# PytorchConnectomics/pytorch_connectomics

Hardware: AMD Instinct MI355X
Metric: voxels/s (train + sliding-window infer), MedNeXt-S 112^3 bf16 (higher is better)
Workload: dtype bf16; 1 GPU; Lucchi++ sliding-window inference (configs[1]): MedNeXt-S k3, 165x1024x768 volume, roi 112^3, overlap 0.5, bump blending, sw_batch_size 8, random-init weights; step = one whole-volume EagerSlidingWindowEngine call (TTA off); value = window-voxels/s; sw_batch_size=8, window_pipeline_streams=3

## Files before the change

include/pytc_hip.h:

```cpp
#ifndef PYTC_HIP_H
#define PYTC_HIP_H

#include <stdint.h>

#ifdef __cplusplus
extern "C" {
#endif

#define PYTC_ABI_VERSION 15

#define PYTC_OK 0
#define PYTC_ERR_INVALID 1
#define PYTC_ERR_HIP 2
#define PYTC_ERR_UNSUPPORTED 3

#define PYTC_F32 0
#define PYTC_BF16 1
#define PYTC_F16 2

#define PYTC_VIEW_FLIP_Z 1
#define PYTC_VIEW_FLIP_Y 2
#define PYTC_VIEW_FLIP_X 4
#define PYTC_VIEW_SWAP_YX 8
#define PYTC_VIEW_SWAP_ZY 16
#define PYTC_VIEW_SWAP_ZX 32

#define PYTC_PAD_CONSTANT 0
#define PYTC_PAD_REFLECT 1
#define PYTC_PAD_REPLICATE 2
#define PYTC_PAD_CIRCULAR 3

#define PYTC_BLEND_PRODUCT 0
#define PYTC_BLEND_MIN 1

#define PYTC_ACT_NONE 0
#define PYTC_ACT_SIGMOID 1
#define PYTC_ACT_TANH 2
#define PYTC_ACT_GELU 3

#define PYTC_RES_NONE 0
#define PYTC_RES_ADD 1
#define PYTC_RES_UPSAMPLE 2
#define PYTC_RES_GELU_BWD 3
#define PYTC_RES_NORM_BWD 4

int pytc_abi_version(void);
const char* pytc_last_error(void);
int pytc_device_info(int device, int* cu_count, int* lds_bytes_per_cu, char* arch, int arch_len);
int pytc_set_tuning(const char* key, int value);


int pytc_gather_windows(const float* vol, int C, int Z, int Y, int X, const int32_t* starts, int B,
                        int rz, int ry, int rx, int view, int pad_mode, float cval, void* out,
                        int out_dtype, void* stream);

int pytc_blend_accumulate(const void* pred, int pred_dtype, int B, const int32_t* starts, int rz,
                          int ry, int rx, int C, int view, const float* wz, const float* wy,
                          const float* wx, int combine, float floor_w, const int32_t* border ,
                          float* value, float* weight, int Z, int Y, int X, void* stream);

int pytc_blend_accumulate_mapped(const void* pred, int pred_dtype, int B, const int32_t* starts, int rz, int ry,
                                 int rx, int C, int view, const float* wz, const float* wy, const float* wx,
                                 int combine, float floor_w, const int32_t* border, const int32_t* chan_src,
                                 const int32_t* chan_shift, float* value, float* weight, int Z, int Y, int X,
                                 void* stream);
int pytc_blend_weight_shifted(int B, const int32_t* starts, int rz, int ry, int rx, const float* wz, const float* wy,
                              const float* wx, int combine, float floor_w, const int32_t* border,
                              const int32_t* shift, float* weight, int Z, int Y, int X, void* stream);
int pytc_normalize_covered(float* value, const float* weight, int64_t n, void* stream);
int pytc_ensemble_update_masked(float* stat, float* count, const float* x, const float* cover, int64_t n, int mode,
                                void* stream);
int pytc_ensemble_finalize_masked(const float* stat, const float* count, float* out, int64_t n, int mode, void* stream);

int pytc_blend_finalize(float* value, const float* weight, int C, int64_t nvox, float clamp,
                        int act, void* stream);

#define PYTC_ACT_SOFTMAX 4
int pytc_channel_activation(float* value, int C, int64_t nvox, int channels_last, int c0, int c1, int act,
                            float scale, void* stream);

int pytc_ensemble_update(float* acc, const float* x, int64_t n, int mode, int count, void* stream);

#define PYTC_ST_U8 0
#define PYTC_ST_I8 1
#define PYTC_ST_U16 2
#define PYTC_ST_I16 3
#define PYTC_ST_I32 4
#define PYTC_ST_F16 5
#define PYTC_ST_F32 6
int pytc_scale_cast(const float* x, void* y, int64_t n, float scale, int target, void* stream);


#define PYTC_RAW_U8 0
#define PYTC_RAW_I8 1
#define PYTC_RAW_U16 2
#define PYTC_RAW_I16 3
#define PYTC_RAW_U32 4
#define PYTC_RAW_I32 5
#define PYTC_RAW_F32 6
#define PYTC_RAW_F64 7
int pytc_resample_region(const void* raw, int raw_dtype, const int64_t* strides_czyx, int C, const int32_t* tab_i0,
                         const int32_t* tab_i1, const float* tab_f, const int32_t* dims_zyx, float* out, void* stream);

#define PYTC_NORM_NONE 0
#define PYTC_NORM_ZSCORE 1
#define PYTC_NORM_MINMAX 2
#define PYTC_NORM_DIVIDE 3
int64_t pytc_window_normalize_ws_elems(int B, int64_t n);
int pytc_window_normalize(float* x, int B, int64_t n, int mode, int binarize, float threshold, float divide, const float* clip,
                          double* workspace, void* stream);


int pytc_dwconv3d_stat_slots(int N, int D, int H, int W, int C, int K, int stride, int dtype,
                             int transposed);

int pytc_dwconv3d_kernel_variant(int N, int D, int H, int W, int C, int K, int stride, int dtype, int transposed);

int pytc_dwconv3d_fwd(const void* x, void* y, const float* w, const float* bias, float* stats,
                      int N, int D, int H, int W, int C, int K, int stride, int dtype,
                      void* stream);

int pytc_dwconv3d_fwd_wide(const void* x, void* y, const float* w, const float* bias, float* stats, int N, int D, int H,
                           int W, int C, int K, int stride, int dtype, void* stream);

int pytc_dwconv3d_res_supported(int D, int H, int W, int C, int K, int stride, int dtype);

int pytc_dwmix_supported(int D, int H, int W, int C, int C_hid, int C_out, int dtype);
int pytc_dwmix_fwd(const void* x, const float* taps, const float* dw_bias, const void* w2n, const float* b2n, const void* w3_f16,
                   const float* b3, int residual, void* y, const void* head_w, const float* head_b, float* head_y, int n_head, int N,
                   int D, int H, int W, int C, int C_hid, int C_out, int dtype, void* stream);
int pytc_dwconv3d_fwd_res(const void* x, const void* res, void* y, const float* w, const float* bias, int N, int D, int H,
                          int W, int C, int K, int stride, int dtype, void* stream);

int pytc_dwconvT3d_fwd(const void* x, void* y, const float* w, const float* bias, float* stats,
                       int N, int D, int H, int W, int C, int K, int dtype, void* stream);

int pytc_groupnorm_finalize(const float* stats, int slots, float count, const float* gamma,
                            const float* beta, float eps, float* ab, int N, int C, void* stream);


int64_t pytc_pw_packed_elems(int C_out, int C_in, int dtype);
int pytc_pw_pack_weight(const float* w, int C_out, int C_in, int transposed, void* packed,
                        int dtype, void* stream);

typedef struct {
  const void* x;
  const void* w_packed;
  const float* bias;
  const float* ab;
  const void* res;
  void* y;
  int N;
  int64_t rows_per_sample;
  int C_in, C_out;
  int in_dtype, out_dtype, w_dtype;
  int act;
  int res_mode;
  int gather;
  int Di, Hi, Wi;
  const void* res_low;
  const float* res_bias;
  int pre_act;
  int w_paired;
} pytc_pw_args;

int pytc_pw_conv_fwd(const pytc_pw_args* a, void* stream);
int pytc_pw_conv_paired_supported(const pytc_pw_args* a);
int pytc_pw_conv_rowmajor_supported(const pytc_pw_args* a);

typedef struct {
  const void* t;
  const float* ab;
  const void* w2_packed;
  const float* b2;
  const void* w3_packed;
  const float* b3;
  const void* res;
  const void* res_low;
  const float* res_bias;
  void* y;
  int N;
  int64_t rows_per_sample;
  int C_in, C_hid, C_out;
  int res_mode;
  int Di, Hi, Wi;
  int w3_format;
  int per_sample;
} pytc_mlp_args;
#define PYTC_W3_BF16 0
#define PYTC_W3_F16 1

int pytc_pw_gemm_supported(int C_in, int C_out);
int pytc_pw_gemm_fwd(const void* x, const void* w, const float* bias, const float* ab, void* y, int N, int64_t rows_per_sample,
                     int C_in, int C_out, int in_f16, int gelu_out, const void* res, const void* res_low, const float* res_bias,
                     int res_mode, int Di, int Hi, int Wi, void* stream);
int pytc_pw_mlp_supported(int C_in, int C_hid, int C_out);
int pytc_pw_pack_weight_paired(const float* w, int C_out, int C_in, int transposed, void* packed_bf16,
                               void* stream);
int pytc_pack_multi(const int64_t* table_dev, int n_items, int64_t total_elems, void* stream);
int pytc_pw_pack_weight_paired_f16(const float* w, int C_out, int C_in, int transposed, void* packed_f16,
                                   void* stream);
int pytc_pw_mlp_fwd(const pytc_mlp_args* a, void* stream);

int pytc_pw_mlp_lds_supported(int C_in, int C_hid, int C_out);
int pytc_pw_mlp_lds_fwd(const pytc_mlp_args* a, void* stream);
int pytc_pw_mlp_dma_applies(const pytc_mlp_args* a, int ignore_res_mode);
int pytc_pw_mlp_proj_supported(int C_in, int C_hid, int C_out, int C_proj);
int pytc_pw_mlp_proj_fwd(const pytc_mlp_args* a, const void* proj_w, const float* proj_b, void* z, int store_y, void* stream);
int pytc_pw_mlp_chunk_supported(int C_in, int C_hid, int C_out);
int pytc_pw_mlp_chunk_fwd(const pytc_mlp_args* a, void* stream);
int pytc_groupnorm_fold_mlp(const float* stats, int slots, float count, const float* gamma, const float* beta, float eps,
                            const float* w2, const float* b2, void* w2n, float* b2n, float* ab_out, int N, int C, int C_hid,
                            void* stream);
int pytc_pw_mlp_train_fwd(const pytc_mlp_args* a, void* hidden_pre, void* stream);
int pytc_pw_mlp_train_fwd_nostore(const pytc_mlp_args* a, void* stream);
int pytc_pw_mlp_bwd(const pytc_mlp_args* a, const void* hidden_pre, void* d_hidden, void* stream);
int pytc_pw_mlp_up_supported(int C_in, int C_hid, int C_out);
int pytc_pw_mlp_up_fwd(const pytc_mlp_args* a, const float* taps, const float* dw_bias, void* stream);
int pytc_pw_mlp_head_supported(int C_in, int C_hid, int C_out);
int pytc_pw_mlp_stemres_fwd(const pytc_mlp_args* a, const float* stem_x, const float* stem_w, const float* stem_b,
                            void* stream);
int pytc_stem_dwconv3d_stat_slots(int D, int H, int W);
int pytc_stem_dwconv3d_supported(int C_in, int C, int K);
int pytc_stem_dwconv3d_mfma_image_bytes(void);
int pytc_stem_dwconv3d_pack_mfma(const float* wx, const float* wb, const float* cst, void* image, void* stream);
int pytc_stem_dwconv3d_fwd(const float* x, const float* wx, const float* wb, const float* cst, const void* mfma_image, void* y,
                           float* stats, int N, int D, int H, int W, int C, void* stream);
int pytc_pw_mlp_head_fwd(const pytc_mlp_args* a, const void* head_w, const float* head_b, float* head_y, int n_head,
                         int store_y, void* stream);


#define PYTC_ACT_RELU 5
#define PYTC_ACT_LEAKY 6
#define PYTC_ACT_ELU 7

typedef struct {
  const void* x;
  const void* w_packed;
  const float* bias;
  const float* ab;
  const void* res;
  void* y;
  int N, D, H, W, C_in, C_out;
  int kd, kh, kw;
  int act_in;
  float act_param;
  int res_mode;
  int dtype;
} pytc_conv3d_args;

int64_t pytc_conv3d_packed_elems(int C_out, int C_in, int kd, int kh, int kw, int dtype);
int pytc_conv3d_pack_weight(const float* w, int C_out, int C_in, int kd, int kh, int kw, void* packed, int dtype,
                            void* stream);
int pytc_conv3d_fwd(const pytc_conv3d_args* a, void* stream);

int pytc_channel_stats_slots(int64_t rows);
int pytc_channel_stats(const void* x, float* stats, int N, int64_t rows, int C, int dtype, void* stream);
int pytc_norm_finalize_groups(const float* stats, int slots, float count, const float* gamma, const float* beta,
                              float eps, int groups, float* ab, int N, int C, void* stream);
int pytc_affine_act(const void* x, void* y, const float* ab, int N, int64_t rows, int C, int act, float prm,
                    int dtype, void* stream);
int pytc_maxpool3d_fwd(const void* x, void* y, int N, int D, int H, int W, int C, int fz, int fy, int fx, int dtype,
                       void* stream);
int pytc_dwconvT3d_generic_fwd(const void* x, void* y, const float* w, int N, int D, int H, int W, int C,
                               const int32_t* kernel, const int32_t* stride, const int32_t* pad, int dtype,
                               void* stream);


int pytc_groupnorm_finalize_mr(const float* stats, int slots, float count, const float* gamma, const float* beta,
                               float eps, float* ab, float* mean_rstd, int N, int C, void* stream);
int pytc_gelu(const void* x, const void* dy, void* out, int64_t n, int dtype, void* stream);
int pytc_add_inplace(void* y, const void* x, int64_t n, int dtype, void* stream);
int pytc_pw_wgrad_slots(int64_t rows_total);
int pytc_pw_wgrad(const void* x, const float* ab, const void* dy, float* dW, float* db, float* workspace, int N,
                  int64_t rows_per_sample, int C_in, int C_out, int dtype, int x_act , void* stream);
int pytc_dw_wgrad_slots(int N, const int32_t* gdims, const int32_t* xdims, int C, int K, int stride, int dtype);
int pytc_dw_wgrad(const void* g, const void* x, float* dW, float* db, float* workspace, int N, const int32_t* gdims,
                  const int32_t* xdims, int C, int K, int stride, int dtype, void* stream);

int pytc_pw_wgrad_partial(const void* x, const float* ab, const void* dy, float* workspace, int want_db, int N,
                          int64_t rows_per_sample, int C_in, int C_out, int dtype, int x_act, int* slots_out, void* stream);
int pytc_pw_wgrad_dgrad_supported(int C_in, int C_out, int dtype);
int pytc_pw_wgrad_dgrad_partial(const void* x, const void* dy, const void* w_t_paired, void* dx, float* workspace, int want_db, int N,
                                int64_t rows_per_sample, int C_in, int C_out, int dtype, int* slots_out, void* stream);
int pytc_mixer_bwd_rc_supported(int C, int C_hid, int C_out, int dtype);
int pytc_mixer_bwd_rc_sps(int N, int64_t rows_per_sample, int C_hid);
int64_t pytc_mixer_bwd_rc_ws_elems(int N, int64_t rows_per_sample, int C_hid, int gn);
int pytc_mixer_bwd_rc(const void* t, const float* ab, const float* mean_rstd, const void* dy, const void* w2_paired, const float* b2,
                      const void* w3t_paired, const float* W2, const float* gamma, float count, void* dhp, float* workspace,
                      float* s_out, float* coef, int want_db3, int gn, int N, int64_t rows_per_sample, int C, int C_hid, int C_out,
                      int dtype, int* slots_out, void* stream);
int pytc_dw_wgrad_partial(const void* g, const void* x, float* workspace, int want_db, int N, const int32_t* gdims,
                          const int32_t* xdims, int C, int K, int stride, int dtype, int* slots_out, void* stream);
int pytc_copy_zero_front(const void* src, void* dst, int N, const int32_t* dims, int C, int dtype, void* stream);
typedef struct {
  const float* part;
  float* out;
  int64_t n;
  int32_t slots;
  int32_t out_t;
} pytc_reduce_item;
int pytc_reduce_slots_multi(const pytc_reduce_item* items, int n_items, void* stream);
int pytc_norm_bwd_ws_elems(int N, int64_t rows, int C);
int pytc_norm_bwd(const void* dtn, const void* t, const float* mean_rstd, const float* gamma, float* stats_ws,
                  float* s_out, void* dt, int N, int64_t rows, float count , int C,
                  int dtype, void* stream);
int pytc_pw_wgrad_groupnorm_supported(int C, int C_hid, int dtype);
int pytc_pw_wgrad_groupnorm_sps(int N, int64_t rows_per_sample, int C, int C_hid);
int64_t pytc_pw_wgrad_groupnorm_ws_elems(int N, int64_t rows_per_sample, int C, int C_hid);
int pytc_pw_wgrad_groupnorm(const void* t, const float* mean_rstd, const float* ab, const void* dhp, const float* W2,
                            const float* gamma, float count, float* s_out, float* coef, float* workspace, int N,
                            int64_t rows_per_sample, int C, int C_hid, int dtype, void* stream);
int pytc_norm_bwd_apply(const void* dtn, const void* t, const float* mean_rstd, const float* gamma, const float* s_in,
                        int s_parts, void* dt, int N, int64_t rows, int C, float count, int dtype, const int32_t* crop_grid,
                        void* stream);
int pytc_dwconv3d_bwd_data(const void* dy, const float* w, void* dx, int N, const int32_t* xdims,
                           const int32_t* ydims, int C, int K, int stride, int dtype, void* stream);
int pytc_dwconv3d_bwd_data_add(const void* dy, const float* w, const void* addend, void* dx, int N, const int32_t* xdims,
                               const int32_t* ydims, int C, int K, int stride, int dtype, void* stream);

int pytc_conv3d_pack_weight_dgrad(const float* w, int C_out, int C_in, int kd, int kh, int kw, void* packed, int dtype,
                                  void* stream);
int pytc_conv3d_pack_plan(int C_out, int C_in, int kd, int kh, int kw, int dtype, int direct, int64_t* out);
int pytc_conv3d_pack_multi(const int64_t* table_dev, int n_items, int64_t total_blocks, void* stream);
int pytc_conv3d_launch_plan(int N, int D, int H, int W, int C_in, int C_out, int kd, int kh, int kw, int dtype, int has_pre,
                            int has_res, int phase, int64_t* out);
int pytc_norm_bwd_means(const float* s, const float* gamma, float* M, float* dgamma, float* dbeta, int N, int C, int groups,
                        float rows, void* stream);
int pytc_bn_train_finalize_cpad(const float* stats, int slots_total, float count, const float* gamma, const float* beta, float eps,
                                float momentum, float* running_mean, float* running_var, int64_t* num_batches_tracked, float* ab,
                                float* mean_rstd, int N, int C, int C_real, void* stream);
int pytc_norm_finalize_groups_cpg(const float* stats, int slots, float count, const float* gamma, const float* beta, float eps,
                                  int groups, int cpg, float* ab, float* mr, int N, int C, void* stream);
int pytc_norm_bwd_means_cpg(const float* s, const float* gamma, float* M, float* dgamma, float* dbeta, int N, int C, int groups,
                            int cpg, float rows, void* stream);
int pytc_bn_train_finalize(const float* stats, int slots_total, float count, const float* gamma, const float* beta, float eps,
                           float momentum, float* running_mean, float* running_var, int64_t* num_batches_tracked, float* ab,
                           float* mean_rstd, int N, int C, void* stream);
int pytc_bn_update_running(const float* mean_rstd, float* running_mean, float* running_var, int C, float count, float eps,
                           float momentum, void* stream);
int64_t pytc_conv3d_wgrad_ws_elems(int N, int D, int H, int W, int C_in, int C_out, const int32_t* kernel, int dtype);
int pytc_conv3d_wgrad(const void* a, const void* dy, float* dW, float* workspace, int N, int D, int H, int W, int C_in,
                      int C_out, const int32_t* kernel, int dtype, void* stream);
int pytc_act_bwd(const void* da, const void* x, const float* ab, void* dt, void* dp, int N, int64_t rows, int C, int act,
                 float prm, int dtype, void* stream);
int pytc_norm_finalize_groups_mr(const float* stats, int slots, float count, const float* gamma, const float* beta,
                                 float eps, int groups, float* ab, float* mr, int N, int C, void* stream);
int pytc_norm_bwd_stats(const void* dtn, const void* t, const float* mean_rstd, float* stats_ws, float* s_out, int N,
                        int64_t rows, int C, int dtype, void* stream);
int pytc_norm_bwd_apply_general(const void* d, const void* x, const float* mean_rstd, const float* gamma, const float* M,
                                void* dx, int N, int64_t rows, int C, int dtype, void* stream);
int pytc_act_norm_bwd_stats(const void* da, const void* x, const float* ab, const float* mean_rstd, float* stats_ws, float* s_out,
                            float* p_ws, float* p_out, int N, int64_t rows, int C, int act, float prm, int dtype, void* stream);
int pytc_act_norm_bwd_apply(const void* da, const void* x, const float* ab, const float* mean_rstd, const float* gamma,
                            const float* M, void* dx, int N, int64_t rows, int C, int act, float prm, int dtype, void* stream);
int pytc_act_norm_bwd_apply_cg(const void* da, const void* x, const float* ab, const float* mean_rstd, const float* gamma, int C_gamma,
                               const float* M, void* dx, int N, int64_t rows, int C, int act, float prm, int dtype, void* stream);
int pytc_maxpool3d_bwd(const void* x, const void* dy, void* dx, int N, int D, int H, int W, int C, int fz, int fy, int fx,
                       int dtype, void* stream);
int pytc_dwconv3d_generic_fwd(const void* x, void* y, const float* w, int N, int D, int H, int W, int C,
                              const int32_t* kernel, const int32_t* stride, const int32_t* pad, const int32_t* out_dims,
                              int dtype, void* stream);

int64_t pytc_conv3d_direct_packed_elems(int C_out, int C_in, int kd, int kh, int kw, int dtype);
int pytc_conv3d_pack_weight_direct(const float* w, int C_out, int C_in, int kd, int kh, int kw, int64_t s_o, int64_t s_c,
                                   int flip, void* packed, int dtype, void* stream);
int pytc_convT3d_c1_fwd(const void* x, const float* w, const float* bias, void* y, float* workspace, int N, const int32_t* in_dims,
                        int C_in, int dtype, void* stream);
int pytc_convT3d_phase_plan(int C_out, int C_in, int dtype, int64_t* out);
int pytc_convT3d_phase_supported(int C_out, int C_in, int dtype);
int pytc_convT3d_phase_fwd(const pytc_conv3d_args* a, const int32_t* in_dims, void* stream);
int pytc_conv3d_strided_fwd(const pytc_conv3d_args* a, const int32_t* in_dims, const int32_t* stride, const int32_t* pad,
                            int transposed, void* stream);
int64_t pytc_conv3d_wgrad_strided_ws_elems(int N, const int32_t* small_dims, int C_k, int C_o, const int32_t* kernel);
int pytc_conv3d_wgrad_strided(const void* big, const void* small, float* dW, float* workspace, int N,
                              const int32_t* big_dims, const int32_t* small_dims, int C_k, int C_o, const int32_t* kernel,
                              const int32_t* stride, const int32_t* pad, int dtype, void* stream);
int pytc_convT3d_thin_supported(int C_in, int C_out);
int pytc_convT3d_thin_fwd(const void* x, const float* w, const float* bias, void* y, int N, const int32_t* in_dims, int C_in,
                          int C_out, int dtype, void* stream);

int pytc_layernorm_rows(const void* x, void* y, const float* gamma, const float* beta, int64_t rows, int C, float eps,
                        int dtype, void* stream);
int pytc_upcat_deconv2_fwd(const void* x_low, const float* w, const float* bias, const void* x_e, void* cat, int N, int d, int h, int wd,
                           int D, int H, int W, int C_in, int C_e, int C_u, int dtype, void* stream);
int pytc_upcat_deconv2_bwd_data(const void* dcat, const float* w, void* dx_e, void* dx_low, int N, int d, int h, int wd, int D, int H,
                                int W, int C_in, int C_e, int C_u, int dtype, void* stream);
int64_t pytc_upcat_deconv2_wgrad_ws_elems(int rows, int C_in, int C_u, int dtype);
int pytc_upcat_deconv2_wgrad(const void* x_low, const void* dcat, float* workspace, float* dw, float* db, int N, int d, int h, int wd,
                             int D, int H, int W, int C_in, int C_e, int C_u, int dtype, void* stream);
int pytc_linear_fwd(const void* x, const float* w, const float* bias, const float* pos, int pos_rows, const void* res, void* y, int M,
                    int N, int K, int x_gelu, int dtype, void* stream);
int pytc_linear_bwd_data(const void* dy, const float* w, const void* x_gelu, void* dx, int M, int N, int K, int dtype, void* stream);
int pytc_linear_wgrad(const void* dy, const void* x, float* dw, float* db, float* dpos, int pos_rows, int M, int N, int K, int x_gelu,
                      int dtype, void* stream);
int pytc_layernorm_wide(const void* x, void* y, const float* gamma, const float* beta, int64_t rows, int C, float eps, int dtype,
                        void* stream);
int pytc_layernorm_wide_bwd_slots(int64_t rows);
int pytc_layernorm_wide_bwd(const void* dy, const void* x, const float* gamma, void* dx, float* partial, float* dgamma, float* dbeta,
                            int64_t rows, int C, float eps, int dtype, void* stream);
int pytc_patch_gather16(const void* src, void* dst, int B, int D, int H, int W, int C, int scatter, int dtype, void* stream);
int pytc_attention_supported(int d_head);
int pytc_attention_fwd(const void* qkv, void* out, float* lse, int B, int N, int heads, int d_head, float scale, int dtype,
                       void* stream);
int pytc_attention_bwd(const void* qkv, const void* out, const void* dout, const float* lse, float* dvec, void* dqkv, int B, int N,
                       int heads, int d_head, float scale, int dtype, void* stream);
int pytc_window_attention_supported(int d_head);
int pytc_window_attention_bias_groups(int nwin, int N, int heads);
int pytc_window_attention_fwd(const void* qkv, const float* table, const int* geom, void* out, float* lse, int nwin, int N, int heads,
                              int d_head, float scale, int dtype, void* stream);
int pytc_window_attention_bwd(const void* qkv, const float* table, const int* geom, const void* out, const void* dout, const float* lse,
                              float* dvec, void* dqkv, float* partial, float* dtable, int nwin, int N, int heads, int d_head, float scale,
                              int dtype, void* stream);
int pytc_window_partition(const void* src, void* dst, const void* res, const int* geom, int B, int C, int reverse, int dtype,
                          void* stream);
int pytc_space_to_depth2(const void* src, void* dst, int B, int D, int H, int W, int C, int order, int scatter, int dtype, void* stream);
int pytc_layernorm_any(const void* x, void* y, const float* gamma, const float* beta, int64_t rows, int C, float eps, int dtype,
                       void* stream);
int pytc_layernorm_any_bwd_slots(int64_t rows);
int pytc_layernorm_any_bwd(const void* dy, const void* x, const float* gamma, void* dx, float* stats, float* partial, float* dgamma,
                           float* dbeta, int64_t rows, int C, float eps, int dtype, void* stream);
int pytc_deconv2_upfirst_fwd(const void* x_low, const float* w, const float* bias, const void* x_e, void* out, int N, int d, int h,
                             int wd, int C_in, int C_e, int C_u, int dtype, void* stream);
int pytc_deconv2_upfirst_bwd_data(const void* dout, const float* w, void* dx_e, void* dx_low, int N, int d, int h, int wd, int C_in,
                                  int C_e, int C_u, int dtype, void* stream);
int pytc_deconv2_upfirst_wgrad(const void* x_low, const void* dout, float* workspace, float* dw, float* db, int N, int d, int h, int wd,
                               int C_in, int C_e, int C_u, int dtype, void* stream);
int pytc_layernorm_rows_bwd_slots(int64_t rows, int C, int dtype);
int pytc_layernorm_rows_bwd(const void* dy, const void* x, const float* gamma, void* dx, float* partial, int64_t rows, int C,
                            float eps, int dtype, void* stream);
int pytc_grn_bwd_apply(const void* dh2, const void* hp, const float* A, const float* B, void* out, int N, int64_t rows, int C,
                       int dtype, void* stream);
int64_t pytc_bce_dice_ws_elems(int N, int C, int64_t R);
int pytc_bce_dice_fwd(const float* logits, const float* target, const float* weight, int N, int C, int64_t R,
                      const int64_t* x_strides, const int64_t* t_strides, const int64_t* w_strides, float pos_weight,
                      float w_bce, float w_dice, float smooth_nr, float smooth_dr, float* workspace, float* sums,
                      float* out, void* stream);
int pytc_bce_dice_bwd(const float* logits, const float* target, const float* weight, const float* sums, const float* out,
// ... 124 lines not shown
```

pytorch_connectomics_amd/csrc/dwconvT_tile_kernels.hip:

```cpp
#include <mutex>

#include "dwconv_march.h"

namespace pytc {

constexpr int TT_TZ = 2, TT_TX = 8;

template <int C, int TY, bool STORE>
__global__ void __launch_bounds__(256, 4)
dwconvT3d_k3_tile_kernel(const unsigned short* __restrict__ x, unsigned short* __restrict__ y, const float* __restrict__ w,
                         const float* __restrict__ bias, float* __restrict__ stats, DwTTile g) {
  constexpr int LPV = C / 2;
  constexpr int SLOTS = 256 / LPV;
  constexpr int CELLS = TT_TZ * TY * TT_TX;
  constexpr int EZ = TT_TZ + 1, EY = TY + 1, EX = TT_TX + 1;
  constexpr int NCH = EZ * EY * EX * (C / 8);
  typedef unsigned int u32x4_t __attribute__((ext_vector_type(4)));
  extern __shared__ __attribute__((aligned(16))) unsigned short tile[];
  unsigned short* const otile = tile + EZ * EY * EX * C + (threadIdx.x >> 6) * 1024;
  __shared__ float red[256 / 64][2][2 * 64];

  const int tid = threadIdx.x;
  int b = blockIdx.x;
  const int fx = b % g.tx; b /= g.tx;
  const int fy = b % g.ty;
  const int fz = b / g.ty;
  const int n = blockIdx.y;
  const int z0 = fz * TT_TZ, y0 = fy * TY, x0 = fx * TT_TX;
  const long vcells = (long)g.D * g.H * g.W;
  const unsigned short* xn = x + (long)n * vcells * C;
  unsigned short* yn = y + (long)n * vcells * 8 * C;
  const int Ho = 2 * g.H, Wo = 2 * g.W;

  constexpr int LPT = (NCH + 255) / 256;
  u32x4_t st[LPT];
#pragma unroll
  for (int i = 0; i < LPT; ++i) {
    const int c = tid + 256 * i;
    const int vox = c / (C / 8), part = c % (C / 8);
    const int lx = vox % EX, t = vox / EX;
    const int ly = t % EY, lz = t / EY;
    const int iz = min(max(z0 - 1 + lz, 0), g.D - 1), iy = min(max(y0 - 1 + ly, 0), g.H - 1), ix = min(max(x0 - 1 + lx, 0), g.W - 1);
    if (c < NCH) st[i] = *reinterpret_cast<const u32x4_t*>(xn + (((long)iz * g.H + iy) * g.W + ix) * C + part * 8);
  }
  const int pr = tid % LPV, slot0 = tid / LPV;
  float wt[27][2];
#pragma unroll
  for (int t = 0; t < 27; ++t) {
    const float2 v = *reinterpret_cast<const float2*>(w + (long)t * C + pr * 2);
    wt[t][0] = v.x; wt[t][1] = v.y;
  }
  float bv[2] = {0.f, 0.f};
  if (bias) { bv[0] = bias[pr * 2]; bv[1] = bias[pr * 2 + 1]; }
#pragma unroll
  for (int i = 0; i < LPT; ++i) {
    const int c = tid + 256 * i;
    if (c < NCH) *reinterpret_cast<u32x4_t*>(tile + (long)c * 8) = st[i];
  }
  __syncthreads();

  typedef __bf16 bf2_t __attribute__((ext_vector_type(2)));
  typedef float f2_t __attribute__((ext_vector_type(2)));
  const unsigned int SX = 2u * C * 2u, SY = (unsigned int)Wo * C * 2u * 2u, SZ = (unsigned int)Ho * Wo * C * 2u * 2u;
  char* const ybase = reinterpret_cast<char*>(yn) + ((((long)2 * z0 * Ho + 2 * y0) * Wo + 2 * x0) * C) * 2;
  const int lane = tid & 63;
  int pcs[2];
  unsigned int poff[2];
#pragma unroll
  for (int k = 0; k < 2; ++k) {
    const int piece = lane + 64 * k, vox = piece / (C / 8), chunk = piece % (C / 8);
    const int q = vox % 8;
    pcs[k] = vox / 8;
    poff[k] = (unsigned int)(q >> 2) * (SZ / 2) + (unsigned int)((q >> 1) & 1) * (SY / 2) + (unsigned int)(q & 1) * (SX / 2) + chunk * 16u;
  }
  const int wslot0 = (tid >> 6) * (64 / LPV);
  f2_t s1 = {0.f, 0.f}, s2 = {0.f, 0.f};
  const bool interior = z0 > 0 && y0 > 0 && x0 > 0 && z0 + TT_TZ <= g.D && y0 + TY <= g.H && x0 + TT_TX <= g.W;
  const f2_t bv2 = {bv[0], bv[1]};
  f2_t wt2[27];
#pragma unroll
  for (int t = 0; t < 27; ++t) wt2[t] = f2_t{wt[t][0], wt[t][1]};
  for (int it = 0; it < CELLS / SLOTS; ++it) {
    const int cell = slot0 + it * SLOTS;
    const int cx = cell % TT_TX, t = cell / TT_TX;
    const int cy = t % TY, cz = t / TY;
    const int mz = z0 + cz, my = y0 + cy, mx = x0 + cx;
    const bool live = interior || (mz < g.D && my < g.H && mx < g.W);
    f2_t xin[2][2][2];
#pragma unroll
    for (int a = 0; a < 2; ++a)
#pragma unroll
      for (int bb = 0; bb < 2; ++bb)
#pragma unroll
        for (int d = 0; d < 2; ++d) {
          const unsigned int v = *reinterpret_cast<const unsigned int*>(tile + ((((cz + a) * EY + cy + bb) * EX + cx + d) * C + pr * 2));
          xin[a][bb][d] = f2_t{__uint_as_float(v << 16), __uint_as_float(v & 0xffff0000u)};
        }
    const bool fz0 = !interior && mz == 0, fy0 = !interior && my == 0, fx0 = !interior && mx == 0;
    unsigned int* const orow = reinterpret_cast<unsigned int*>(otile) + ((slot0 - wslot0) * 8) * (C / 2) + pr;
#pragma unroll
    for (int pz = 0; pz < 2; ++pz)
#pragma unroll
      for (int py = 0; py < 2; ++py)
#pragma unroll
        for (int px = 0; px < 2; ++px) {
          f2_t acc = bv2;
#pragma unroll
          for (int a = pz; a < 2; ++a)
#pragma unroll
            for (int bb = py; bb < 2; ++bb)
#pragma unroll
              for (int d = px; d < 2; ++d) {
                const int kz = pz ? 1 : (a ? 0 : 2), ky = py ? 1 : (bb ? 0 : 2), kx = px ? 1 : (d ? 0 : 2);
                acc = __builtin_elementwise_fma(xin[a][bb][d], wt2[(kz * 3 + ky) * 3 + kx], acc);
              }
          const bool zero = !live || (pz == 0 && fz0) || (py == 0 && fy0) || (px == 0 && fx0);
          unsigned int bits = __builtin_bit_cast(unsigned int, __builtin_convertvector(acc, bf2_t));
          bits = zero ? 0u : bits;
          if (STORE) orow[(pz * 4 + py * 2 + px) * (C / 2)] = bits;
          const f2_t r = {__uint_as_float(bits << 16), __uint_as_float(bits & 0xffff0000u)};
          s1 += r;
          s2 = __builtin_elementwise_fma(r, r, s2);
        }
    if (STORE) {
      __builtin_amdgcn_wave_barrier();
#pragma unroll
      for (int k = 0; k < 2; ++k) {
        const u32x4_t o = *reinterpret_cast<const u32x4_t*>(otile + (lane + 64 * k) * 8);
        const int c2 = wslot0 + pcs[k] + it * SLOTS;
        const int c2x = c2 % TT_TX, t2 = c2 / TT_TX;
        const int c2y = t2 % TY, c2z = t2 / TY;
        const bool ok = interior || (z0 + c2z < g.D && y0 + c2y < g.H && x0 + c2x < g.W);
        const unsigned int off = __umul24((unsigned int)c2z, SZ) + __umul24((unsigned int)c2y, SY) + (unsigned int)c2x * SX + poff[k];
        if (ok) *reinterpret_cast<u32x4_t*>(ybase + off) = o;
      }
      __builtin_amdgcn_wave_barrier();
    }
  }
  if (stats) {
    if (LPV == 32) {
#pragma unroll
      for (int i = 0; i < 2; ++i) { s1[i] += __shfl_xor(s1[i], 32, 64); s2[i] += __shfl_xor(s2[i], 32, 64); }
    }
    const int wave = tid >> 6, lane = tid & 63;
    if (lane < LPV) {
      red[wave][0][(lane % LPV) * 2] = s1[0]; red[wave][0][(lane % LPV) * 2 + 1] = s1[1];
      red[wave][1][(lane % LPV) * 2] = s2[0]; red[wave][1][(lane % LPV) * 2 + 1] = s2[1];
    }
    __syncthreads();
    if (tid < 2 * C) {
      const int which = tid / C, ch = tid % C;
      float a = 0.f;
#pragma unroll
      for (int wv = 0; wv < 4; ++wv) a += red[wv][which][ch];
      stats[(((long)n * g.slots + blockIdx.x) * 2 + which) * C + ch] = a;
    }
  }
}

bool dwconvT_tile_plan(DwTTile& g, int N, int D, int H, int W, int C) {
  if (C != 64 && C != 128) return false;
  const int ty = C == 64 ? 8 : 4;
  g.N = N; g.D = D; g.H = H; g.W = W; g.C = C;
  g.tz = (D + TT_TZ - 1) / TT_TZ; g.ty = (H + ty - 1) / ty; g.tx = (W + TT_TX - 1) / TT_TX;
  g.slots = g.tz * g.ty * g.tx;
  return g.slots >= 1 && (long)D * H * W * 8 * C * 2 < (1L << 32) && (long)(2 * H) * (2 * W) * C * 4 < (1L << 24);
}

void dwconvT_tile_launch(const void* x, void* y, const float* w, const float* bias, float* stats, const DwTTile& g, hipStream_t s) {
  dim3 grid((unsigned)g.slots, (unsigned)g.N), block(256);
  const unsigned short* xp = (const unsigned short*)x;
  unsigned short* yp = (unsigned short*)y;
#define PYTC_TT(CC, TYY, ST)                                                                                                  \
  do {                                                                                                                        \
    if (!ensure_dynamic_lds(reinterpret_cast<const void*>(&dwconvT3d_k3_tile_kernel<CC, TYY, ST>), 64 * 1024, "dwconvT3d_k3_tile")) return; \
    hipLaunchKernelGGL((dwconvT3d_k3_tile_kernel<CC, TYY, ST>), grid, block,                                                  \
                       (size_t)(TT_TZ + 1) * (TYY + 1) * (TT_TX + 1) * CC * 2 + 4 * 2048, s, xp, yp, w, bias, stats, g);                  \
  } while (0)
  if (g.C == 64) { if (y) PYTC_TT(64, 8, true); else PYTC_TT(64, 8, false); }
  else { if (y) PYTC_TT(128, 4, true); else PYTC_TT(128, 4, false); }
#undef PYTC_TT
}

}
```

pytorch_connectomics_amd/csrc/dwconv_march.h:

```cpp
#pragma once
#include "pytc_common.h"

namespace pytc {

struct DwMarch {
  int N, D, H, W, C;
  int ty, tx, zc, nzc;
  int tilex;
  int slots;
  int swizzle;
  int cg_inner;
};

void dwconv_mfma_launch(const void* x, void* y, const float* w, const float* bias, float* stats, const DwMarch& g, int variant,
                        hipStream_t s);

struct DwMix {
  const bf16x8_t* w2n;
  const float* b2n;
  const h8_t* w3;
  const float* b3;
  long w2_stride;
  int residual;
  const bf16x8_t* head_w;
  const float* head_b;
  float* head_y;
  int n_head, store_y;
};
int dwmix_launch(const void* x, void* y, const float* w, const float* bias, const DwMarch& g, const DwMix& mx, int c_hid, int variant,
                 hipStream_t s);

struct DwTTile { int N, D, H, W, C, tz, ty, tx, slots; };
bool dwconvT_tile_plan(DwTTile& g, int N, int D, int H, int W, int C);
void dwconvT_tile_launch(const void* x, void* y, const float* w, const float* bias, float* stats, const DwTTile& g, hipStream_t s);

struct DwS2 { int N, D, H, W, C, Do, Ho, Wo, ty, tx, zc, nzc, slots; };
bool dwconv_s2_plan(DwS2& g, int N, int D, int H, int W, int C);
void dwconv_s2_launch(const void* x, void* y, const float* w, const float* bias, float* stats, const DwS2& g, hipStream_t s);

}
```

pytorch_connectomics_amd/csrc/dwconv_s2_kernels.hip:

```cpp
#include <mutex>

#include "dwconv_march.h"

namespace pytc {

constexpr int S2_TYO = 4;

template <int C>
__global__ void __launch_bounds__(256, 2)
dwconv3d_k3_s2_march_kernel(const unsigned short* __restrict__ x, unsigned short* __restrict__ y, const float* __restrict__ w,
                            const float* __restrict__ bias, float* __restrict__ stats, DwS2 g) {
  constexpr int TYO = S2_TYO, TXO = 8, IY = 2 * TYO + 1, IX = 2 * TXO + 1;
  constexpr int LPV = C / 2, VS = 256 / LPV, OUTV = TYO * TXO, ITEMS = OUTV / VS;
  constexpr int PCH = IY * IX * (C / 8);
  constexpr int LPT = (PCH + 255) / 256;
  constexpr int PLANE = IY * IX * C;
  typedef unsigned int u32x4_t __attribute__((ext_vector_type(4)));
  typedef float f2_t __attribute__((ext_vector_type(2)));
  typedef __bf16 bf2_t __attribute__((ext_vector_type(2)));
  constexpr int OPIECES = OUTV * C / 8;
  static_assert(OUTV % VS == 0 && OPIECES <= 256, "at most one 16-byte output piece per thread and plane");
  extern __shared__ __attribute__((aligned(16))) unsigned short ring[];
  unsigned short* const otile = ring + 3 * PLANE;
  __shared__ float red[4][2][2 * 64];

  const int tid = threadIdx.x;
  int b = blockIdx.x;
  const int fx = b % g.tx; b /= g.tx;
  const int fy = b % g.ty;
  const int zchunk = b / g.ty;
  const int n = blockIdx.y;
  const int yo0 = fy * TYO, xo0 = fx * TXO;
  const int zs = zchunk * g.zc, ze = min(zs + g.zc, g.Do);
  const long in_plane = (long)g.H * g.W * C;
  const unsigned short* xn = x + (long)n * g.D * in_plane;
  unsigned short* yn = y + (long)n * g.Do * g.Ho * g.Wo * C;

  int goff[LPT], loff[LPT];
  bool cok[LPT];
#pragma unroll
  for (int i = 0; i < LPT; ++i) {
    const int c = tid + 256 * i;
    const int vox = c / (C / 8), part = c % (C / 8);
    const int lx = vox % IX, ly = vox / IX;
    const int iy = 2 * yo0 - 1 + ly, ix = 2 * xo0 - 1 + lx;
    cok[i] = c < PCH && iy >= 0 && iy < g.H && ix >= 0 && ix < g.W;
    goff[i] = (min(max(iy, 0), g.H - 1) * g.W + min(max(ix, 0), g.W - 1)) * C + part * 8;
    loff[i] = c < PCH ? c * 8 : -1;
  }
  auto request = [&](int iz, u32x4_t (&st)[LPT]) {
    const unsigned short* src = xn + (long)min(max(iz, 0), g.D - 1) * in_plane;
#pragma unroll
    for (int i = 0; i < LPT; ++i) st[i] = *reinterpret_cast<const u32x4_t*>(src + goff[i]);
  };
  auto deposit = [&](int iz, const u32x4_t (&st)[LPT]) {
    const bool zok = iz >= 0 && iz < g.D;
    unsigned short* dst = ring + ((iz + 1) % 3) * PLANE;
#pragma unroll
    for (int i = 0; i < LPT; ++i)
      if (loff[i] >= 0) *reinterpret_cast<u32x4_t*>(dst + loff[i]) = (zok && cok[i]) ? st[i] : u32x4_t{0u, 0u, 0u, 0u};
  };

  const int pr = tid % LPV, vslot = tid / LPV;
  f2_t wt[27];
#pragma unroll
  for (int t = 0; t < 27; ++t) {
    const float2 v = *reinterpret_cast<const float2*>(w + (long)t * C + pr * 2);
    wt[t] = f2_t{v.x, v.y};
  }
  f2_t bv = {0.f, 0.f};
  if (bias) bv = f2_t{bias[pr * 2], bias[pr * 2 + 1]};
  const int ovx = tid / (C / 8), opart = tid % (C / 8);
  const int oyy = yo0 + ovx / TXO, oxx = xo0 + ovx % TXO;
  const bool ook = tid < OPIECES && oyy < g.Ho && oxx < g.Wo;
  const long obase = ((long)oyy * g.Wo + oxx) * C + opart * 8;

  u32x4_t sa[LPT], sb[LPT];
  request(2 * zs - 1, sa);
  request(2 * zs, sb);
  deposit(2 * zs - 1, sa);
  deposit(2 * zs, sb);
  request(2 * zs + 1, sa);
  deposit(2 * zs + 1, sa);
  __syncthreads();

  f2_t s1 = {0.f, 0.f}, s2 = {0.f, 0.f};
  for (int zo = zs; zo < ze; ++zo) {
    const bool more = zo + 1 < ze;
    if (more) { request(2 * zo + 2, sa); request(2 * zo + 3, sb); }
    const unsigned short* p0 = ring + ((2 * zo) % 3) * PLANE;
    const unsigned short* p1 = ring + ((2 * zo + 1) % 3) * PLANE;
    const unsigned short* p2 = ring + ((2 * zo + 2) % 3) * PLANE;
#pragma unroll
    for (int it = 0; it < ITEMS; ++it) {
      const int v = vslot + it * VS;
      const int vy = v / TXO, vx = v % TXO;
      const int base = ((2 * vy) * IX + 2 * vx) * C + pr * 2;
      f2_t acc = bv;
#pragma unroll
      for (int kz = 0; kz < 3; ++kz) {
        const unsigned short* pl = kz == 0 ? p0 : (kz == 1 ? p1 : p2);
#pragma unroll
        for (int ky = 0; ky < 3; ++ky)
#pragma unroll
          for (int kx = 0; kx < 3; ++kx) {
            const unsigned int u = *reinterpret_cast<const unsigned int*>(pl + base + (ky * IX + kx) * C);
            acc = __builtin_elementwise_fma(f2_t{__uint_as_float(u << 16), __uint_as_float(u & 0xffff0000u)}, wt[(kz * 3 + ky) * 3 + kx], acc);
          }
      }
      const bool live = (yo0 + vy) < g.Ho && (xo0 + vx) < g.Wo;
      unsigned int bits = __builtin_bit_cast(unsigned int, __builtin_convertvector(acc, bf2_t));
      bits = live ? bits : 0u;
      reinterpret_cast<unsigned int*>(otile)[v * (C / 2) + pr] = bits;
      const f2_t r = {__uint_as_float(bits << 16), __uint_as_float(bits & 0xffff0000u)};
      s1 += r;
      s2 = __builtin_elementwise_fma(r, r, s2);
    }
    __syncthreads();
    const u32x4_t o = *reinterpret_cast<const u32x4_t*>(otile + (tid < OPIECES ? tid : 0) * 8);
    if (ook) *reinterpret_cast<u32x4_t*>(yn + (long)zo * g.Ho * g.Wo * C + obase) = o;
    if (more) { deposit(2 * zo + 2, sa); deposit(2 * zo + 3, sb); }
    __syncthreads();
  }

  if (stats) {
#pragma unroll
    for (int off = LPV; off < 64; off <<= 1) {
#pragma unroll
      for (int i = 0; i < 2; ++i) { s1[i] += __shfl_xor(s1[i], off, 64); s2[i] += __shfl_xor(s2[i], off, 64); }
    }
    const int wave = tid >> 6, lane = tid & 63;
    if (lane < LPV) {
      red[wave][0][lane * 2] = s1[0]; red[wave][0][lane * 2 + 1] = s1[1];
      red[wave][1][lane * 2] = s2[0]; red[wave][1][lane * 2 + 1] = s2[1];
    }
    __syncthreads();
    if (tid < 2 * C) {
      const int which = tid / C, ch = tid % C;
      float a = 0.f;
#pragma unroll
      for (int wv = 0; wv < 4; ++wv) a += red[wv][which][ch];
      stats[(((long)n * g.slots + blockIdx.x) * 2 + which) * C + ch] = a;
    }
  }
}

bool dwconv_s2_plan(DwS2& g, int N, int D, int H, int W, int C) {
  if (C != 32 && C != 64) return false;
  constexpr int tyo = S2_TYO;
  g.N = N; g.D = D; g.H = H; g.W = W; g.C = C;
  g.Do = (D - 1) / 2 + 1; g.Ho = (H - 1) / 2 + 1; g.Wo = (W - 1) / 2 + 1;
  g.ty = (g.Ho + tyo - 1) / tyo; g.tx = (g.Wo + 7) / 8;
  int nzc = (128 + g.ty * g.tx - 1) / (g.ty * g.tx);
  const int maxc = g.Do / 7 < 1 ? 1 : g.Do / 7;
  if (nzc > maxc) nzc = maxc;
  if (nzc < 1) nzc = 1;
  g.zc = (g.Do + nzc - 1) / nzc;
  g.nzc = (g.Do + g.zc - 1) / g.zc;
  g.slots = g.ty * g.tx * g.nzc;
  return (long)H * W * C < (1L << 30);
}

void dwconv_s2_launch(const void* x, void* y, const float* w, const float* bias, float* stats, const DwS2& g, hipStream_t s) {
  dim3 grid((unsigned)g.slots, (unsigned)g.N), block(256);
  const unsigned short* xp = (const unsigned short*)x;
  unsigned short* yp = (unsigned short*)y;
#define PYTC_S2(CC)                                                                                                           \
  do {                                                                                                                        \
    const size_t lds = (size_t)(3 * (2 * S2_TYO + 1) * 17 * CC + S2_TYO * 8 * CC) * 2;                                         \
    if (!ensure_dynamic_lds(reinterpret_cast<const void*>(&dwconv3d_k3_s2_march_kernel<CC>), 72 * 1024, "dwconv3d_k3_s2_march")) return; \
    hipLaunchKernelGGL((dwconv3d_k3_s2_march_kernel<CC>), grid, block, lds, s, xp, yp, w, bias, stats, g);                    \
  } while (0)
  if (g.C == 32) PYTC_S2(32);
  else PYTC_S2(64);
#undef PYTC_S2
}

}
```

pytorch_connectomics_amd/csrc/pytc_common.h:

```cpp
#pragma once
#include <hip/hip_runtime.h>
#include <stdint.h>
#include <stdio.h>
#include <string.h>

#include "../../include/pytc_hip.h"

namespace pytc {

typedef __bf16 bf16_t;
typedef __bf16 bf16x2_t __attribute__((ext_vector_type(2)));
typedef __bf16 bf16x4_t __attribute__((ext_vector_type(4)));
typedef __bf16 bf16x8_t __attribute__((ext_vector_type(8)));
typedef float f32x2_t __attribute__((ext_vector_type(2)));
typedef float f32x4_t __attribute__((ext_vector_type(4)));
typedef float f32x8_t __attribute__((ext_vector_type(8)));
typedef float f32x16_t __attribute__((ext_vector_type(16)));
typedef short s16x8_t __attribute__((ext_vector_type(8)));

constexpr int WAVE = 64;

void set_error(const char* fmt, ...);
int hip_fail(hipError_t e, const char* what);
bool ensure_dynamic_lds(const void* kernel, size_t bytes, const char* what);
bool take_launch_failure();

#define PYTC_REQUIRE(cond, ...)                     \
  do {                                              \
    if (!(cond)) {                                  \
      pytc::set_error(__VA_ARGS__);                 \
      return PYTC_ERR_INVALID;                      \
    }                                               \
  } while (0)

#define PYTC_LAUNCH_CHECK(name)                                  \
  do {                                                           \
    if (pytc::take_launch_failure()) return PYTC_ERR_HIP;        \
    hipError_t e_ = hipGetLastError();                           \
    if (e_ != hipSuccess) return pytc::hip_fail(e_, name);       \
  } while (0)

#define PYTC_CHECK_DTYPE(dtype, what) \
  PYTC_REQUIRE((dtype) == PYTC_BF16 || (dtype) == PYTC_F32, "%s: bad dtype %d", what, (int)(dtype))

#define PYTC_DISPATCH_DTYPE(dtype, what, T, ...)      \
  do {                                                \
    if ((dtype) == PYTC_BF16) {                       \
      using T = pytc::bf16_t;                         \
      __VA_ARGS__;                                    \
    } else if ((dtype) == PYTC_F32) {                 \
      using T = float;                                \
      __VA_ARGS__;                                    \
    } else {                                          \
      PYTC_CHECK_DTYPE(dtype, what);                  \
    }                                                 \
  } while (0)

constexpr int elems_per_16b(int dtype) { return dtype == PYTC_BF16 ? 8 : 4; }
constexpr int mfma_kstep(int dtype) { return dtype == PYTC_BF16 ? 32 : 16; }
template <typename T>
constexpr int elems_per_16b_of = 16 / (int)sizeof(T);
static_assert(elems_per_16b_of<__bf16> == elems_per_16b(PYTC_BF16) && elems_per_16b_of<float> == elems_per_16b(PYTC_F32), "one width rule");

#define PYTC_KNOBS(X)                                                                                                             \
  X(channel_act_flat, 1, "channel activation of contiguous NDHWC tensors as a flat 16-byte stream; 0 = the per-voxel kernel")      \
  X(conv_wgrad_mfma, 1, "dense-conv weight gradient on the matrix cores (bf16); 0 = the VALU kernel")                              \
  X(dw_wgrad_march, 1, "depthwise K = 3 / stride 1 weight gradient as a z-march; 0 = the vector / generic kernels")                \
  X(dw_wgrad_vec, 1, "depthwise K = 3 weight gradient with 16-byte channel vectors; 0 = the generic kernel")                       \
  X(dwconvT_tile, 1, "transposed depthwise conv at C = 64 / 128 (bf16) as one tile of input cells per workgroup; 0 = cell kernel") \
  X(dwconv_march_h16, 1, "VALU z-march depthwise conv: packed-f16 in-plane partial sums; 0 = fp32 taps")                           \
  X(dwconv_mfma, 1, "bf16 stride-1 K = 3 depthwise forward (and the fused block) on the matrix cores; 0 = the VALU z-march")       \
  X(dwconv_mfma_variant, 0, "matrix-core depthwise conv: bit 0 = hi + lo weight halves, bit 1 = two planes in flight, not three")  \
  X(dwconv_s2_march, 1, "stride-2 K = 3 depthwise conv at C = 32 / 64 (bf16) as a z-march over an LDS ring; 0 = gather kernel")    \
  X(elementwise_vec, 1, "16-byte vector forms of the norm-apply / elementwise training kernels; 0 = the scalar kernels")           \
  X(mixer_bwd_rc_slot_div, 1, "recomputing mixer backward: divide the slot count (fewer, longer slots)")                           \
  X(mlp_chunk_variant, 0, "chunked-hidden mixer (pw_mlp_chunk_kernels.hip): tile shape of the launch")                             \
  X(mlp_dma, 1, "level-0 mixer with DMA-prefetched row tiles (pw_mlp_dma_kernel); 0 = one tile per wave")                          \
  X(mlp_dma_rows, 1 << 20, "fewest rows of a launch that takes the DMA mixer")                                                     \
  X(mlp_dma_wgs, 0, "DMA mixer: workgroups per sample; 0 = chosen from the row count")                                             \
  X(mlp_lds_variant, 0, "LDS-resident mixer (pw_mlp_lds_kernels.hip): tile shape of the launch")                                   \
  X(norm_bwd_from_wgrad_flat, 1, "GroupNorm-backward epilogue of the expand weight gradient as one flat kernel; 0 = chunked")      \
  X(pw_gemm_rows, 0, "LDS-tiled 1x1 GEMM: 64 / 128 forces the rows per workgroup; 0 = by problem size")                            \
  X(pw_thin, 1, "plain 1x1 convs with one input / few output channels on the thin kernels; 0 = the generic kernel")                \
  X(wgrad_dgrad_fused, 1, "projecting conv's weight gradient and the GELU-backward data gradient in one kernel; 0 = two launches")  \
  X(wgrad_small_split, 1, "matrix-core 1x1 weight gradient: more, shorter row slots when the launch would leave CUs idle")         \
  X(wgrad_valu, 0, "1: 1x1 weight gradient on the VALU kernel instead of the matrix cores")                                        \
  X(wgrad_whole_rounds, 1, "matrix-core 1x1 weight gradient: round the slot count down to whole rounds of resident workgroups")

enum Knob {
#define PYTC_KNOB_ENUM(name, dflt, doc) K_##name,
  PYTC_KNOBS(PYTC_KNOB_ENUM)
#undef PYTC_KNOB_ENUM
  K_COUNT
};
int tuning_get(Knob k);

template <typename T, int VEC>
struct VecIO;

template <int VEC>
struct VecIO<float, VEC> {
  typedef float vec_t __attribute__((ext_vector_type(VEC)));
  static __device__ __forceinline__ void load(const float* p, float (&v)[VEC]) {
    vec_t t = *reinterpret_cast<const vec_t*>(p);
#pragma unroll
    for (int i = 0; i < VEC; ++i) v[i] = t[i];
  }
  static __device__ __forceinline__ void store(float* p, const float (&v)[VEC]) {
    vec_t t;
#pragma unroll
    for (int i = 0; i < VEC; ++i) t[i] = v[i];
    *reinterpret_cast<vec_t*>(p) = t;
  }
};
template <>
struct VecIO<float, 1> {
  static __device__ __forceinline__ void load(const float* p, float (&v)[1]) { v[0] = *p; }
  static __device__ __forceinline__ void store(float* p, const float (&v)[1]) { *p = v[0]; }
};

template <int VEC>
struct VecIO<bf16_t, VEC> {
  typedef __bf16 vec_t __attribute__((ext_vector_type(VEC)));
  typedef float fvec_t __attribute__((ext_vector_type(VEC)));
  static __device__ __forceinline__ void load(const bf16_t* p, float (&v)[VEC]) {
    vec_t t = *reinterpret_cast<const vec_t*>(p);
    fvec_t f = __builtin_convertvector(t, fvec_t);
#pragma unroll
    for (int i = 0; i < VEC; ++i) v[i] = f[i];
  }
  static __device__ __forceinline__ void store(bf16_t* p, const float (&v)[VEC]) {
    fvec_t f;
#pragma unroll
    for (int i = 0; i < VEC; ++i) f[i] = v[i];
    *reinterpret_cast<vec_t*>(p) = __builtin_convertvector(f, vec_t);
  }
};
template <>
struct VecIO<bf16_t, 1> {
  static __device__ __forceinline__ void load(const bf16_t* p, float (&v)[1]) { v[0] = (float)*p; }
  static __device__ __forceinline__ void store(bf16_t* p, const float (&v)[1]) { *p = (bf16_t)v[0]; }
};

template <typename T>
__device__ __forceinline__ float to_f32(T v) { return (float)v; }
template <typename T>
__device__ __forceinline__ T from_f32(float v) { return (T)v; }

__device__ __forceinline__ float wave_sum(float v) {
#pragma unroll
  for (int o = 32; o > 0; o >>= 1) v += __shfl_xor(v, o, 64);
  return v;
}

template <int THREADS, typename T>
__device__ __forceinline__ T block_sum(T v, T* red) {
  red[threadIdx.x] = v;
  __syncthreads();
  for (int s = THREADS / 2; s > 0; s >>= 1) {
    if ((int)threadIdx.x < s) red[threadIdx.x] += red[threadIdx.x + s];
    __syncthreads();
  }
  const T r = red[0];
  __syncthreads();
  return r;
}

__device__ __forceinline__ float gelu_erf(float x) {
  const float az = fabsf(x) * 0.70710678118654752440f;
  const float t = __builtin_amdgcn_rcpf(fmaf(0.3275911f, az, 1.0f));
  float p = fmaf(t, 1.061405429f, -1.453152027f);
  p = fmaf(t, p, 1.421413741f);
  p = fmaf(t, p, -0.284496736f);
  p = fmaf(t, p, 0.254829592f);
  p *= t;
  const float e = __builtin_amdgcn_exp2f(-az * az * 1.44269504088896340736f);
  const float one_plus_erf = x < 0.f ? p * e : fmaf(-p, e, 2.0f);
  return 0.5f * x * one_plus_erf;
}

__device__ __forceinline__ float gelu_erf_grad(float x) {
  const float az = fabsf(x) * 0.70710678118654752440f;
  const float t = __builtin_amdgcn_rcpf(fmaf(0.3275911f, az, 1.0f));
  float p = fmaf(t, 1.061405429f, -1.453152027f);
  p = fmaf(t, p, 1.421413741f);
  p = fmaf(t, p, -0.284496736f);
  p = fmaf(t, p, 0.254829592f);
  p *= t;
  const float e = __builtin_amdgcn_exp2f(-az * az * 1.44269504088896340736f);
  const float one_plus_erf = x < 0.f ? p * e : fmaf(-p, e, 2.0f);
  return fmaf(x * 0.3989422804014327f, e, 0.5f * one_plus_erf);
}

__device__ __forceinline__ float gelu_grad(float x) {
  const float phi_big = 0.5f * (1.0f + erff(x * 0.70710678118654752440f));
  const float pdf = 0.3989422804014327f * __expf(-0.5f * x * x);
  return phi_big + x * pdf;
}

__device__ __forceinline__ float gelu_fast(float x) {
  const float x2 = fminf(x * x, 64.0f);
  float p = fmaf(x2, 1.0142630e-3f, -1.0677572e-1f);
  p = fmaf(p, x2, -2.3011213f);
  const float e = __builtin_amdgcn_exp2f(x * p);
  return x * __builtin_amdgcn_rcpf(1.0f + e);
}

__device__ __forceinline__ void gelu_fast_with_grad(float x, float& g, float& gd) {
  const float x2 = fminf(x * x, 64.0f);
  float p = fmaf(x2, 1.0142630e-3f, -1.0677572e-1f);
  p = fmaf(p, x2, -2.3011213f);
  const float e = __builtin_amdgcn_exp2f(x * p);
  const float s = __builtin_amdgcn_rcpf(1.0f + e);
  g = x * s;
  const float q = fmaf(x2, 2.0f * 1.0142630e-3f, -1.0677572e-1f);
  const float du = fmaf(x2 + x2, q, p);
  gd = fmaf(g * (1.0f - s), du * -0.69314718055994530942f, s);
}

typedef _Float16 h2_t __attribute__((ext_vector_type(2)));
typedef _Float16 h8_t __attribute__((ext_vector_type(8)));

__device__ __forceinline__ h2_t gelu_h2(h2_t x) {
  const h2_t U = {(_Float16)3.75f, (_Float16)3.75f};
  const h2_t u = __builtin_elementwise_min(__builtin_elementwise_abs(x), U);
  const h2_t t = u * (h2_t){(_Float16)(2.0f / 3.75f), (_Float16)(2.0f / 3.75f)} + (h2_t){(_Float16)-1.0f, (_Float16)-1.0f};
#define PYTC_H2C(v) ((h2_t){(_Float16)(v), (_Float16)(v)})
  h2_t p = PYTC_H2C(-6.166994737e-02f);
  p = p * t + PYTC_H2C(6.367329291e-02f);
  p = p * t + PYTC_H2C(1.683184914e-01f);
  p = p * t + PYTC_H2C(-3.056981228e-01f);
  p = p * t + PYTC_H2C(7.903670132e-02f);
  p = p * t + PYTC_H2C(1.852329106e-01f);
  p = p * t + PYTC_H2C(-1.855973189e-01f);
  p = p * t + PYTC_H2C(5.694380662e-02f);
#undef PYTC_H2C
  return __builtin_elementwise_max(x, (h2_t){(_Float16)0.0f, (_Float16)0.0f}) - p;
}

__device__ __forceinline__ h8_t gelu_h8_from_f32(const float (&v)[8]) {
#define PYTC_H2C(c) ((h2_t){(_Float16)(c), (_Float16)(c)})
  h2_t x[4], t[4], p[4];
#pragma unroll
  for (int q = 0; q < 4; ++q) x[q] = __builtin_bit_cast(h2_t, __builtin_amdgcn_cvt_pkrtz(v[2 * q], v[2 * q + 1]));
#pragma unroll
  for (int q = 0; q < 4; ++q) t[q] = __builtin_elementwise_min(__builtin_elementwise_abs(x[q]), PYTC_H2C(3.75f));
#pragma unroll
  for (int q = 0; q < 4; ++q) t[q] = t[q] * PYTC_H2C(2.0f / 3.75f) + PYTC_H2C(-1.0f);
#pragma unroll
  for (int q = 0; q < 4; ++q) p[q] = PYTC_H2C(-6.166994737e-02f) * t[q] + PYTC_H2C(6.367329291e-02f);
#define PYTC_STEP(c)                                                    \
  _Pragma("unroll") for (int q = 0; q < 4; ++q) p[q] = p[q] * t[q] + PYTC_H2C(c);
  PYTC_STEP(1.683184914e-01f)
  PYTC_STEP(-3.056981228e-01f)
  PYTC_STEP(7.903670132e-02f)
  PYTC_STEP(1.852329106e-01f)
  PYTC_STEP(-1.855973189e-01f)
  PYTC_STEP(5.694380662e-02f)
#undef PYTC_STEP
  h8_t out;
#pragma unroll
  for (int q = 0; q < 4; ++q) {
    const h2_t g = __builtin_elementwise_max(x[q], PYTC_H2C(0.0f)) - p[q];
    out[2 * q] = g[0];
    out[2 * q + 1] = g[1];
  }
#undef PYTC_H2C
  return out;
}

__device__ __forceinline__ int xcd_swizzle(int b, int nblocks) {
  const int q = nblocks >> 3, r = nblocks & 7;
  const int xcd = b & 7, idx = b >> 3;
  return (xcd < r ? xcd * (q + 1) : r * (q + 1) + (xcd - r) * q) + idx;
}

static inline int ceil_div(long a, long b) { return (int)((a + b - 1) / b); }

}
```

pytorch_connectomics_amd/hip_ops.py:

```python
from __future__ import annotations

import ctypes as C
from typing import Optional, Sequence

import torch

from . import _native as nat

_DT = {torch.float32: nat.F32, torch.bfloat16: nat.BF16}


def dtype_code(dt: torch.dtype) -> int:
    try:
        return _DT[dt]
    except KeyError:
        raise TypeError(f"pytorch_connectomics_amd kernels support float32/bfloat16, got {dt}") from None


def require_device(device, what: str = "this inference path") -> None:
    if torch.device(device).type != "cuda":
        raise RuntimeError(f"{what} (pytorch_connectomics_amd) needs a CUDA(HIP) device: there is no CPU path")


def _on_device(t: torch.Tensor, name: str) -> torch.Tensor:
    if not isinstance(t, torch.Tensor) or not t.is_cuda:
        raise RuntimeError(f"{name} must be a CUDA(HIP) tensor: pytorch_connectomics_amd has no CPU path")
    return t


def _dev(t: torch.Tensor, name: str) -> torch.Tensor:
    _on_device(t, name)
    if not t.is_contiguous():
        raise RuntimeError(f"{name} must be contiguous")
    return t


def _p(t: Optional[torch.Tensor]):
    return C.c_void_p(t.data_ptr()) if t is not None else None


_raw_stream = getattr(torch._C, "_cuda_getCurrentRawStream", None)
_raw_device = getattr(torch._C, "_cuda_getDevice", None)


def _stream():
    if _raw_stream is not None and _raw_device is not None:
        return C.c_void_p(_raw_stream(_raw_device()))
    return C.c_void_p(torch.cuda.current_stream().cuda_stream)


class _Profiler:
    def __init__(self):
        self.enabled = False
        self.records = []

    def summary(self):
        torch.cuda.synchronize()
        out = {}
        for name, s, e, nbytes, flops, symbol in self.records:
            d = out.setdefault(name, {"launches": 0, "ms": 0.0, "bytes": 0, "flops": 0, "symbol": symbol})
            d["launches"] += 1
            d["ms"] += s.elapsed_time(e)
            d["bytes"] += nbytes
            d["flops"] += flops
        return out

    def by_symbol(self):
        torch.cuda.synchronize()
        out = {}
        for name, s, e, nbytes, flops, symbol in self.records:
            d = out.setdefault(symbol, {"launches": 0, "ms": 0.0, "bytes": 0, "flops": 0, "labels": []})
            d["launches"] += 1
            d["ms"] += s.elapsed_time(e)
            d["bytes"] += nbytes
            d["flops"] += flops
            if name not in d["labels"]:
                d["labels"].append(name)
        return out


PROFILER = _Profiler()


class profiled:

    def __enter__(self):
        PROFILER.records = []
        PROFILER.enabled = True
        return PROFILER

    def __exit__(self, *exc):
        PROFILER.enabled = False
        return False


def _run(name: str, nbytes: int, fn, *args, flops: int = 0, symbol: Optional[str] = None) -> None:
    if PROFILER.enabled:
        s = torch.cuda.Event(enable_timing=True)
        e = torch.cuda.Event(enable_timing=True)
        s.record()
        st = fn(*args)
        e.record()
        PROFILER.records.append((name, s, e, int(nbytes), int(flops), symbol or name.split("[")[0]))
    else:
        st = fn(*args)
    nat.check(st, name)


def _nbytes(*ts) -> int:
    return sum(t.numel() * t.element_size() for t in ts if t is not None)


def _starts_array(starts: Sequence[Sequence[int]], windows: Optional[int] = None):
    if windows is not None and len(starts) != int(windows):
        raise ValueError(f"{int(windows)} window predictions for {len(starts)} window positions: the network must keep the batch size")
    flat = [int(v) for s in starts for v in s]
    return (C.c_int32 * len(flat))(*flat)


def _f32_operand(t, name: str, *, shape=None, numel: Optional[int] = None) -> None:
    if not isinstance(t, torch.Tensor) or not t.is_cuda or t.dtype != torch.float32 or not t.is_contiguous():
        raise ValueError(f"{name} must be a contiguous float32 CUDA(HIP) tensor")
    if shape is not None and tuple(t.shape) != tuple(shape):
        raise ValueError(f"{name} must have shape {tuple(shape)}, got {tuple(t.shape)}")
    if numel is not None and t.numel() != numel:
        raise ValueError(f"{name} must have {numel} elements, got {t.numel()}")


def _window_operands(name: str, roi, weight, wshape, wz, wy, wx) -> None:
    for t, n, ax in ((wz, roi[0], "wz"), (wy, roi[1], "wy"), (wx, roi[2], "wx")):
        _f32_operand(t, f"{name}: {ax}", shape=(int(n),))
    if weight is not None:
        _f32_operand(weight, f"{name}: weight", shape=wshape)


def gather_windows(vol: torch.Tensor, starts, roi, *, view: int = 0, pad_mode: str = "constant",
                   cval: float = 0.0, out_dtype: torch.dtype = torch.float32,
                   out: Optional[torch.Tensor] = None) -> torch.Tensor:
    _dev(vol, "vol")
    if vol.dtype != torch.float32 or vol.dim() != 4:
        raise ValueError("vol must be float32 with shape (C, Z, Y, X)")
    Cc, Z, Y, X = vol.shape
    B = len(starts)
    rz, ry, rx = (int(v) for v in roi)
    if out is None:
        out = torch.empty((B, rz, ry, rx, Cc), dtype=out_dtype, device=vol.device)
    elif (not isinstance(out, torch.Tensor) or not out.is_cuda or not out.is_contiguous() or out.dtype not in _DT
          or tuple(out.shape) != (B, rz, ry, rx, Cc)):
        raise ValueError(f"gather_windows: out must be a contiguous float32 / bfloat16 CUDA(HIP) tensor of shape {(B, rz, ry, rx, Cc)}")
    st = _starts_array(starts)
    for b0 in range(0, B, 64):
        nb = min(64, B - b0)
        sub = (C.c_int32 * (3 * nb)).from_buffer(st, 4 * 3 * b0)
        o = out[b0:b0 + nb]
        _run("gather_windows", 2 * _nbytes(o) if o.dtype == torch.float32 else 3 * _nbytes(o),
             nat.lib().pytc_gather_windows, _p(vol), Cc, Z, Y, X, sub, nb, rz, ry, rx, int(view),
             nat.PAD_MODES[pad_mode], float(cval), _p(o), dtype_code(out.dtype), _stream())
    return out


def blend_accumulate(pred: torch.Tensor, starts, value: torch.Tensor, weight: Optional[torch.Tensor],
                     wz: torch.Tensor, wy: torch.Tensor, wx: torch.Tensor, *, view: int = 0,
                     combine: int = nat.BLEND_PRODUCT, floor_w: float = 1e-5, border=None) -> None:
    _dev(pred, "pred"); _dev(value, "value")
    B, rz, ry, rx, Cc = pred.shape
    if value.dtype != torch.float32 or value.shape[0] != Cc:
        raise ValueError("value accumulator must be float32 (C, Z, Y, X) with C matching pred")
    _, Z, Y, X = value.shape
    _window_operands("blend_accumulate", (rz, ry, rx), weight, (Z, Y, X), wz, wy, wx)
    st = _starts_array(starts, B)
    bd = (C.c_int32 * 3)(*[int(v) for v in border]) if border else None
    win = B * rz * ry * rx
    _run("blend_accumulate", _nbytes(pred) + win * 4 * (2 * Cc + (2 if weight is not None else 0)),
         nat.lib().pytc_blend_accumulate, _p(pred), dtype_code(pred.dtype), B, st, rz, ry, rx, Cc, int(view),
         _p(wz), _p(wy), _p(wx), int(combine), float(floor_w), bd, _p(value), _p(weight), Z, Y, X, _stream())


def blend_accumulate_mapped(pred: torch.Tensor, starts, value: torch.Tensor, weight: Optional[torch.Tensor],
                            wz: torch.Tensor, wy: torch.Tensor, wx: torch.Tensor, chan_src, chan_shift, *, view: int = 0,
                            combine: int = nat.BLEND_PRODUCT, floor_w: float = 1e-5, border=None) -> None:
    _dev(pred, "pred"); _dev(value, "value")
    B, rz, ry, rx, Cc = pred.shape
    if value.dtype != torch.float32 or value.shape[0] != Cc:
        raise ValueError("value accumulator must be float32 (C, Z, Y, X) with C matching pred")
    if len(chan_src) != Cc or len(chan_shift) != Cc:
        raise ValueError("channel map must describe every output channel")
    _, Z, Y, X = value.shape
    _window_operands("blend_accumulate_mapped", (rz, ry, rx), weight, (Z, Y, X), wz, wy, wx)
    st = _starts_array(starts, B)
    bd = (C.c_int32 * 3)(*[int(v) for v in border]) if border else None
    cs = (C.c_int32 * Cc)(*[int(v) for v in chan_src])
    sh = (C.c_int32 * (3 * Cc))(*[int(v) for s3 in chan_shift for v in s3])
    win = B * rz * ry * rx
    _run("blend_accumulate_mapped", _nbytes(pred) + win * 4 * (2 * Cc + (2 if weight is not None else 0)),
         nat.lib().pytc_blend_accumulate_mapped, _p(pred), dtype_code(pred.dtype), B, st, rz, ry, rx, Cc, int(view),
         _p(wz), _p(wy), _p(wx), int(combine), float(floor_w), bd, cs, sh, _p(value), _p(weight), Z, Y, X, _stream())


def blend_weight_shifted(starts, roi, weight: torch.Tensor, wz, wy, wx, shift, *, combine: int = nat.BLEND_PRODUCT,
                         floor_w: float = 1e-5, border=None) -> None:
    _on_device(weight, "weight")
    if weight.dim() != 3 or len(roi) != 3 or len(shift) != 3:
        raise ValueError("blend_weight_shifted: weight must be (Z, Y, X), roi and shift three integers")
    Z, Y, X = weight.shape
    _window_operands("blend_weight_shifted", roi, weight, (Z, Y, X), wz, wy, wx)
    st = _starts_array(starts)
    B = len(starts)
    bd = (C.c_int32 * 3)(*[int(v) for v in border]) if border else None
    sh = (C.c_int32 * 3)(*[int(v) for v in shift])
    _run("blend_weight_shifted", B * int(roi[0]) * int(roi[1]) * int(roi[2]) * 8, nat.lib().pytc_blend_weight_shifted, B, st,
         int(roi[0]), int(roi[1]), int(roi[2]), _p(wz), _p(wy), _p(wx), int(combine), float(floor_w), bd, sh, _p(weight),
         Z, Y, X, _stream())


def normalize_covered(value: torch.Tensor, weight: torch.Tensor) -> None:
    _dev(value, "value"); _dev(weight, "weight")
    if value.numel() != weight.numel() or value.dtype != torch.float32 or weight.dtype != torch.float32:
        raise ValueError("normalize_covered expects float32 tensors of equal size")
    _run("normalize_covered", 2 * _nbytes(value) + _nbytes(weight), nat.lib().pytc_normalize_covered, _p(value), _p(weight),
         value.numel(), _stream())


def ensemble_update_masked(stat: torch.Tensor, count: torch.Tensor, x: torch.Tensor, cover: Optional[torch.Tensor],
                           mode: int) -> None:
    n = stat.numel()
    for t, name in ((stat, "stat"), (count, "count"), (x, "x")) + (((cover, "cover"),) if cover is not None else ()):
        _on_device(t, name)
        _f32_operand(t, f"ensemble_update_masked: {name}", numel=n)
    _run("ensemble_update_masked", 3 * _nbytes(stat) + 2 * _nbytes(count), nat.lib().pytc_ensemble_update_masked, _p(stat),
         _p(count), _p(x), _p(cover), stat.numel(), int(mode), _stream())


def ensemble_finalize_masked(stat: torch.Tensor, count: torch.Tensor, out: torch.Tensor, mode: int) -> None:
    n = stat.numel()
    for t, name in ((stat, "stat"), (count, "count"), (out, "out")):
        _on_device(t, name)
        _f32_operand(t, f"ensemble_finalize_masked: {name}", numel=n)
    _run("ensemble_finalize_masked", 3 * _nbytes(stat), nat.lib().pytc_ensemble_finalize_masked, _p(stat), _p(count), _p(out),
         stat.numel(), int(mode), _stream())


def blend_finalize(value: torch.Tensor, weight: torch.Tensor, *, clamp: float = 1e-4, act: int = nat.ACT_NONE) -> None:
    _on_device(value, "value"); _on_device(weight, "weight")
    Cc = value.shape[0]
    nvox = weight.numel()
    _f32_operand(weight, "blend_finalize: weight")
    _f32_operand(value, "blend_finalize: value", numel=Cc * nvox)
    _run("blend_finalize", 2 * _nbytes(value) + _nbytes(weight), nat.lib().pytc_blend_finalize, _p(value),
         _p(weight), Cc, nvox, float(clamp), int(act), _stream())


def channel_activation(value: torch.Tensor, c0: int, c1: int, act: int, scale: float = 1.0, *,
                       channels_last: bool = False) -> None:
    _dev(value, "value")
    if value.dtype != torch.float32:
        raise TypeError("channel_activation works on float32 volumes")
    Cc = value.shape[-1] if channels_last else value.shape[0]
    nvox = value.numel() // Cc
    _run("channel_activation", 2 * nvox * 4 * (c1 - c0), nat.lib().pytc_channel_activation, _p(value), Cc, nvox,
         int(channels_last), int(c0), int(c1), int(act), float(scale), _stream())


def ensemble_update(acc: torch.Tensor, x: torch.Tensor, mode: int, count: int) -> None:
    _on_device(acc, "acc"); _on_device(x, "x")
    _f32_operand(acc, "ensemble_update: acc")
    _f32_operand(x, "ensemble_update: x", numel=acc.numel())
    _run("ensemble_update", 2 * _nbytes(acc) + _nbytes(x), nat.lib().pytc_ensemble_update, _p(acc), _p(x),
         acc.numel(), int(mode), int(count), _stream())


def resample_region(raw_bytes: torch.Tensor, raw_dtype: str, strides_czyx, channels: int, tab_i0: torch.Tensor,
                    tab_i1: torch.Tensor, tab_f: torch.Tensor, dims_zyx) -> torch.Tensor:
    _dev(raw_bytes, "raw_bytes"); _dev(tab_i0, "tab_i0"); _dev(tab_i1, "tab_i1"); _dev(tab_f, "tab_f")
    if raw_dtype not in nat.RAW_DTYPES:
        raise TypeError(f"resample_region: stored dtype {raw_dtype} is not supported (one of {sorted(nat.RAW_DTYPES)})")
    nz, ny, nx = (int(v) for v in dims_zyx)
    n = nz + ny + nx
    if tab_i0.numel() != n or tab_i1.numel() != n or tab_f.numel() != n or tab_i0.dtype != torch.int32 or tab_f.dtype != torch.float32:
        raise ValueError("resample_region: tables must be int32 / int32 / float32 vectors of nz + ny + nx entries")
    out = torch.empty((int(channels), nz, ny, nx), dtype=torch.float32, device=raw_bytes.device)
    st = (C.c_int64 * 4)(*[int(v) for v in strides_czyx])
    _run("resample_region", raw_bytes.numel() + _nbytes(out), nat.lib().pytc_resample_region, _p(raw_bytes), nat.RAW_DTYPES[raw_dtype],
         st, int(channels), _p(tab_i0), _p(tab_i1), _p(tab_f), _i3((nz, ny, nx)), _p(out), _stream())
    return out


def window_normalize(x: torch.Tensor, *, mode: int = nat.NORM_NONE, binarize: bool = False, threshold: float = 0.0,
                     divide: float = 1.0, clip: Optional[torch.Tensor] = None) -> torch.Tensor:
    _dev(x, "x")
    if x.dtype != torch.float32:
        raise TypeError("window_normalize works on float32 windows")
    B = int(x.shape[0])
    n = x.numel() // max(B, 1)
    if clip is not None:
        _dev(clip, "clip")
        if tuple(clip.shape) != (B, 2) or clip.dtype != torch.float32:
            raise ValueError("window_normalize: clip must be float32 (B, 2)")
    ws = None
    if mode in (nat.NORM_ZSCORE, nat.NORM_MINMAX):
        ws = torch.empty((int(nat.lib().pytc_window_normalize_ws_elems(B, n)),), dtype=torch.float64, device=x.device)
    _run("window_normalize", 2 * _nbytes(x) * (2 if ws is not None else 1), nat.lib().pytc_window_normalize, _p(x), B, n, int(mode),
         int(bool(binarize)), float(threshold), float(divide), _p(clip), _p(ws), _stream())
    return x


def dwconv3d(x: torch.Tensor, w_taps: torch.Tensor, bias: Optional[torch.Tensor], *, K: int, stride: int = 1,
             stats: bool = True, transposed: bool = False, y: Optional[torch.Tensor] = None, store: bool = True,
             wide_range: bool = False):
    _dev(x, "x"); _dev(w_taps, "w_taps")
    N, D, H, W, Cc = x.shape
    dt = dtype_code(x.dtype)
    if transposed:
        oshape = (N, 2 * D, 2 * H, 2 * W, Cc)
    else:
        p = K // 2
        oshape = (N, (D + 2 * p - K) // stride + 1, (H + 2 * p - K) // stride + 1, (W + 2 * p - K) // stride + 1, Cc)
    if not store:
        if not (K == 3 and stats and (transposed or (stride == 1 and x.dtype == torch.bfloat16))):
            raise ValueError("dwconv3d(store=False) is the statistics-only mode of the K = 3 transposed / bf16 stride-1 convs")
        y = None
    elif y is None:
        y = torch.empty(oshape, dtype=x.dtype, device=x.device)
    st = None
    if stats:
        slots = nat.lib().pytc_dwconv3d_stat_slots(N, D, H, W, Cc, K, stride, dt, int(transposed))
        if slots < 0:
            raise RuntimeError(f"dwconv3d: unsupported channel count {Cc}")
        st = torch.empty((N, slots, 2, Cc), dtype=torch.float32, device=x.device)
    tag = f"C{Cc}_k{K}" + ("_s2" if stride == 2 and not transposed else "")
    if transposed:
        _run(f"dwconvT3d_fwd[{tag}]" if store else f"dwconvT3d_stats[{tag}]", _nbytes(x, y), nat.lib().pytc_dwconvT3d_fwd, _p(x), _p(y), _p(w_taps), _p(bias),
             _p(st), N, D, H, W, Cc, K, dt, _stream())
    else:
        sym = None
        if PROFILER.enabled:
            sym = _DW_VARIANTS.get(nat.lib().pytc_dwconv3d_kernel_variant(N, D, H, W, Cc, K, stride, dt, 0))
        fn = nat.lib().pytc_dwconv3d_fwd_wide if wide_range else nat.lib().pytc_dwconv3d_fwd
        _run(f"dwconv3d_fwd[{tag}]" if store else f"dwconv3d_stats[{tag}]", _nbytes(x, y), fn, _p(x), _p(y), _p(w_taps), _p(bias),
             _p(st), N, D, H, W, Cc, K, stride, dt, _stream(), symbol=sym)
    return y, st


_DW_VARIANTS = {0: "dwconv3d_direct_kernel", 1: "dwconv3d_k3_gather_kernel", 2: "dwconv3d_xblock_kernel",
                3: "dwconv3d_k3_march_kernel", 4: "dwconvT3d_k3_cell_kernel", 5: "dwconvT3d_kernel",
                6: "dwconv3d_k3_mfma_kernel", 7: "dwconvT3d_k3_tile_kernel", 8: "dwconv3d_k3_s2_march_kernel"}


def dwconv3d_res_supported(x: torch.Tensor, K: int, stride: int = 1) -> bool:
    N, D, H, W, Cc = x.shape
    return bool(nat.lib().pytc_dwconv3d_res_supported(D, H, W, Cc, K, stride, dtype_code(x.dtype)))


def dwconv3d_res(x: torch.Tensor, w_taps: torch.Tensor, res: torch.Tensor, *, K: int = 3) -> torch.Tensor:
    _dev(x, "x"); _dev(res, "res"); _dev(w_taps, "w_taps")
    if res.shape != x.shape or res.dtype != x.dtype:
        raise ValueError("dwconv3d_res: the residual must match the (stride-1) output shape and dtype")
    N, D, H, W, Cc = x.shape
    y = torch.empty_like(x)
    _run(f"dwconv3d_res[C{Cc}_k{K}]", _nbytes(x, y, res), nat.lib().pytc_dwconv3d_fwd_res, _p(x), _p(res), _p(y), _p(w_taps), None,
         N, D, H, W, Cc, K, 1, dtype_code(x.dtype), _stream(), symbol="dwconv3d_k3_march_kernel")
    return y


def layernorm_rows(x: torch.Tensor, gamma: Optional[torch.Tensor], beta: Optional[torch.Tensor], eps: float = 1e-5) -> torch.Tensor:
    _dev(x, "x")
    Cc = x.shape[-1]
    y = torch.empty_like(x)
    _run(f"layernorm_rows[C{Cc}]", 2 * _nbytes(x), nat.lib().pytc_layernorm_rows, _p(x), _p(y), _p(gamma), _p(beta),
         x.numel() // Cc, Cc, float(eps), dtype_code(x.dtype), _stream())
    return y


def layernorm_rows_bwd(dy: torch.Tensor, x: torch.Tensor, gamma: Optional[torch.Tensor], eps: float = 1e-5):
    _dev(dy, "dy"); _dev(x, "x")
    Cc = x.shape[-1]
    rows = x.numel() // Cc
    slots = nat.lib().pytc_layernorm_rows_bwd_slots(rows, Cc, dtype_code(x.dtype))
    if slots <= 0:
        raise ValueError(f"layernorm_rows_bwd: unsupported channel count {Cc}")
    dx = torch.empty_like(x)
    partial = torch.empty((slots, 2, Cc), dtype=torch.float32, device=x.device)
    _run(f"layernorm_rows_bwd[C{Cc}]", _nbytes(dy, x, dx), nat.lib().pytc_layernorm_rows_bwd, _p(dy), _p(x), _p(gamma), _p(dx),
         _p(partial), rows, Cc, float(eps), dtype_code(x.dtype), _stream())
    return dx, partial


def grn_bwd_apply(dh2: torch.Tensor, hp: torch.Tensor, A: torch.Tensor, B: torch.Tensor) -> torch.Tensor:
    _dev(dh2, "dh2"); _dev(hp, "hp")
    N, Cc = hp.shape[0], hp.shape[-1]
    rows = hp.numel() // (N * Cc)
    out = torch.empty_like(hp)
    _run(f"grn_bwd_apply[C{Cc}]", _nbytes(dh2, hp, out), nat.lib().pytc_grn_bwd_apply, _p(dh2), _p(hp), _p(A), _p(B), _p(out), N,
         rows, Cc, dtype_code(hp.dtype), _stream())
    return out


def groupnorm_finalize(stats: torch.Tensor, count: float, gamma: Optional[torch.Tensor],
                       beta: Optional[torch.Tensor], eps: float = 1e-5) -> torch.Tensor:
    N, slots, _, Cc = stats.shape
    ab = torch.empty((N, 2, Cc), dtype=torch.float32, device=stats.device)
    _run("groupnorm_finalize", _nbytes(stats, ab), nat.lib().pytc_groupnorm_finalize, _p(stats), slots, float(count),
         _p(gamma), _p(beta), float(eps), _p(ab), N, Cc, _stream())
    return ab


def groupnorm_fold_mlp_supported(c: int, c_hid: int) -> bool:
    return c in (32, 64, 128) and c_hid % 32 == 0 and 32 <= c_hid <= 512


def groupnorm_fold_mlp(stats: torch.Tensor, count: float, gamma: Optional[torch.Tensor], beta: Optional[torch.Tensor], eps: float,
                       w2: torch.Tensor, b2: Optional[torch.Tensor], *, want_ab: bool = False):
    N, slots, _, Cc = stats.shape
    c_hid = int(w2.shape[0])
    if w2.dtype != torch.float32 or tuple(w2.shape) != (c_hid, Cc) or not w2.is_contiguous():
        raise ValueError(f"groupnorm_fold_mlp: w2 must be contiguous fp32 (C_hid, {Cc}), got {tuple(w2.shape)} {w2.dtype}")
    w2n = torch.empty((N, c_hid * Cc), dtype=torch.bfloat16, device=stats.device)
    b2n = torch.empty((N, c_hid), dtype=torch.float32, device=stats.device)
    ab = torch.empty((N, 2, Cc), dtype=torch.float32, device=stats.device) if want_ab else None
    _run("groupnorm_finalize", _nbytes(stats, w2n, b2n), nat.lib().pytc_groupnorm_fold_mlp, _p(stats), slots, float(count),
         _p(gamma), _p(beta), float(eps), _p(w2), _p(b2), _p(w2n), _p(b2n), _p(ab), N, Cc, c_hid, _stream())
    return (w2n, b2n, ab) if want_ab else (w2n, b2n)


def pw_pack_weight(w: torch.Tensor, dtype: torch.dtype, *, transposed: bool = False) -> torch.Tensor:
    _dev(w, "w")
    if w.dtype != torch.float32 or w.dim() != 2:
        raise ValueError("pointwise weight must be float32 2-D")
    c_out, c_in = (w.shape[1], w.shape[0]) if transposed else (w.shape[0], w.shape[1])
    n = nat.lib().pytc_pw_packed_elems(c_out, c_in, dtype_code(dtype))
    packed = torch.empty((n,), dtype=dtype, device=w.device)
    _run("pw_pack_weight", _nbytes(w, packed), nat.lib().pytc_pw_pack_weight, _p(w), c_out, c_in, int(transposed),
         _p(packed), dtype_code(dtype), _stream())
    return packed


def pw_conv(x: torch.Tensor, w_packed: torch.Tensor, bias: Optional[torch.Tensor], *, N: int, rows_per_sample: int,
            c_in: int, c_out: int, out_dtype: torch.dtype, ab: Optional[torch.Tensor] = None,
            act: int = nat.ACT_NONE, res: Optional[torch.Tensor] = None, res_mode: int = nat.RES_NONE,
            gather: int = 0, grid: Sequence[int] = (0, 0, 0), res_low: Optional[torch.Tensor] = None,
            res_bias: Optional[torch.Tensor] = None, y: Optional[torch.Tensor] = None,
            pre_act: int = nat.ACT_NONE, w_paired=False) -> torch.Tensor:
    _dev(x, "x"); _dev(w_packed, "w_packed")
    if y is None:
        y = torch.empty((N, rows_per_sample, c_out), dtype=out_dtype, device=x.device)
    a = nat.PwArgs()
    a.x, a.w_packed, a.bias, a.ab, a.res, a.y = (x.data_ptr(), w_packed.data_ptr(),
                                                 bias.data_ptr() if bias is not None else None,
                                                 ab.data_ptr() if ab is not None else None,
                                                 res.data_ptr() if res is not None else None, y.data_ptr())
    a.N, a.rows_per_sample, a.C_in, a.C_out = N, rows_per_sample, c_in, c_out
    a.in_dtype, a.out_dtype, a.w_dtype = dtype_code(x.dtype), dtype_code(y.dtype), dtype_code(w_packed.dtype)
    a.act, a.res_mode, a.gather, a.pre_act, a.w_paired = act, res_mode, gather, pre_act, int(w_paired)
    a.Di, a.Hi, a.Wi = (int(v) for v in grid)
    a.res_low = res_low.data_ptr() if res_low is not None else None
    a.res_bias = res_bias.data_ptr() if res_bias is not None else None
    rows_in = N * rows_per_sample * c_in * x.element_size()
    nb = rows_in + _nbytes(y) + (_nbytes(y) if res is not None else 0)
    _run(f"pw_conv_fwd[{c_in}->{c_out}]", nb, nat.lib().pytc_pw_conv_fwd, C.byref(a), _stream(),
         **({"symbol": "pw_gemm_lds_kernel"} if int(w_paired) == 2 else {}))
    return y


def pw_conv_paired_supported(*, c_in: int, c_out: int, in_dtype: torch.dtype, out_dtype: torch.dtype,
                             w_dtype: torch.dtype = torch.bfloat16, act: int = nat.ACT_NONE, gather: int = 0) -> bool:
    a = nat.PwArgs()
    a.C_in, a.C_out, a.act, a.gather = int(c_in), int(c_out), int(act), int(gather)
    try:
        a.in_dtype, a.out_dtype, a.w_dtype = dtype_code(in_dtype), dtype_code(out_dtype), dtype_code(w_dtype)
    except Exception:
        return False
    return bool(nat.lib().pytc_pw_conv_paired_supported(C.byref(a)))


def _mlp_symbol(a, plain: str, kind: int) -> str:
    if not PROFILER.enabled:
        return plain
    if nat.lib().pytc_pw_mlp_dma_applies(C.byref(a), 1 if kind == 1 else 0):
        return f"pw_mlp_dma_kernel<{int(a.C_hid) // 32}, {kind}>"
    return plain


def pw_mlp_supported(c_in: int, c_hid: int, c_out: int) -> bool:
    return bool(nat.lib().pytc_pw_mlp_supported(int(c_in), int(c_hid), int(c_out)))


MLP_F16_PROJECT = True


def pw_pack_weight_paired(w: torch.Tensor, *, transposed: bool = False, f16: bool = False) -> torch.Tensor:
    _dev(w, "w")
    if w.dtype != torch.float32 or w.dim() != 2:
        raise ValueError("pointwise weight must be float32 2-D")
    c_out, c_in = (w.shape[1], w.shape[0]) if transposed else (w.shape[0], w.shape[1])
    n = nat.lib().pytc_pw_packed_elems(c_out, c_in, nat.BF16)
    packed = torch.empty((n,), dtype=torch.float16 if f16 else torch.bfloat16, device=w.device)
    fn = nat.lib().pytc_pw_pack_weight_paired_f16 if f16 else nat.lib().pytc_pw_pack_weight_paired
    _run("pw_pack_weight_paired", _nbytes(w, packed), fn, _p(w), c_out, c_in, int(transposed), _p(packed), _stream())
    return packed


PACK_PAIRED, PACK_PAIRED_T, PACK_PAIRED_F16, PACK_PAIRED_F16_T, PACK_TAPS, PACK_TAPS_FLIPPED, PACK_ROWMAJOR, PACK_ROWMAJOR_T = range(8)


class StepPacks:

    def __init__(self):
        self.rows = []
        self.index = {}
        self.table = None
        self.total = 0

    def lookup(self, w: torch.Tensor, kind: int):
        i = self.index.get((w.data_ptr(), kind))
        if i is None:
            return None
        row = self.rows[i]
        return row[1] if row[7] == w._version else None

    def register(self, w: torch.Tensor, kind: int, out: torch.Tensor, c_out: int, c_in: int, aux: int) -> None:
        key = (w.data_ptr(), kind)
        i = self.index.get(key)
        row = [w, out, int(kind), int(c_out), int(c_in), int(aux), int(out.numel()), w._version]
        if i is None:
            self.index[key] = len(self.rows)
            self.rows.append(row)
        else:
            self.rows[i] = row
        self.table = None

    def refresh(self) -> None:
        if not self.rows or all(r[7] == r[0]._version for r in self.rows):
            return
        dev = self.rows[0][1].device
        if self.table is None:
            flat, pos = [], 0
            for src, out, kind, c_out, c_in, aux, n, _ver in self.rows:
                flat += [src.data_ptr(), out.data_ptr(), kind, c_out, c_in, aux, pos, n]
                pos += n
            self.table = torch.tensor(flat, dtype=torch.int64).to(dev)
            self.total = pos
        _run("pack_multi", self.total * 6, nat.lib().pytc_pack_multi, _p(self.table), len(self.rows), self.total, _stream())
        for r in self.rows:
            r[7] = r[0]._version


def packed_paired(w_mat: torch.Tensor, *, transposed: bool = False, f16: bool = False, packs: Optional[StepPacks] = None):
    if packs is None:
        return pw_pack_weight_paired(w_mat, transposed=transposed, f16=f16)
    kind = (PACK_PAIRED_F16 if f16 else PACK_PAIRED) + (1 if transposed else 0)
    hit = packs.lookup(w_mat, kind)
    if hit is not None:
        return hit
    out = pw_pack_weight_paired(w_mat, transposed=transposed, f16=f16)
    c_out, c_in = (w_mat.shape[1], w_mat.shape[0]) if transposed else (w_mat.shape[0], w_mat.shape[1])
    packs.register(w_mat, kind, out, c_out, c_in, (c_in + 31) // 32)
    return out


def packed_rowmajor(w_mat: torch.Tensor, *, transposed: bool = False, packs: Optional[StepPacks] = None) -> torch.Tensor:
    kind = PACK_ROWMAJOR_T if transposed else PACK_ROWMAJOR
    if packs is not None:
        hit = packs.lookup(w_mat, kind)
        if hit is not None:
            return hit
    out = (w_mat.t() if transposed else w_mat).to(torch.bfloat16).contiguous()
    if packs is not None:
        c_out, c_in = (w_mat.shape[1], w_mat.shape[0]) if transposed else (w_mat.shape[0], w_mat.shape[1])
        packs.register(w_mat, kind, out, c_out, c_in, 0)
    return out


def pw_conv_rowmajor_supported(*, c_in: int, c_out: int, in_dtype: torch.dtype, out_dtype: torch.dtype, act: int = nat.ACT_NONE,
                               gather: int = 0) -> bool:
    a = nat.PwArgs()
    a.C_in, a.C_out, a.act, a.gather = int(c_in), int(c_out), int(act), int(gather)
    try:
        a.in_dtype, a.out_dtype, a.w_dtype = dtype_code(in_dtype), dtype_code(out_dtype), dtype_code(torch.bfloat16)
    except Exception:
        return False
    return bool(nat.lib().pytc_pw_conv_rowmajor_supported(C.byref(a)))


def packed_taps(w: torch.Tensor, *, flipped: bool = False, packs: Optional[StepPacks] = None) -> torch.Tensor:
    c, k3 = w.shape[0], w.shape[-1] ** 3
    src = w.detach()
    kind = PACK_TAPS_FLIPPED if flipped else PACK_TAPS
    if packs is not None and src.dtype == torch.float32 and src.is_contiguous():
        hit = packs.lookup(src, kind)
        if hit is not None:
            return hit
    out = src.float().reshape(c, k3).t().contiguous()
    if flipped:
        out = torch.flip(out, dims=[0]).contiguous()
    if packs is not None and src.dtype == torch.float32 and src.is_contiguous():
        packs.register(src, kind, out, c, 1, k3)
    return out


def _check_out(y: torch.Tensor, numel: int, dtype: torch.dtype, what: str) -> None:
    _dev(y, "y")
    if y.dtype != dtype or y.numel() != numel or not y.is_contiguous():
        raise ValueError(f"{what}: output buffer must be a contiguous {dtype} tensor of {numel} elements, got "
                         f"{tuple(y.shape)} {y.dtype} contiguous={y.is_contiguous()}")


def _w3_format(w3p: torch.Tensor) -> int:
    return nat.W3_F16 if w3p.dtype == torch.float16 else nat.W3_BF16


def _folded_operands(ab, w2p: torch.Tensor, b2: torch.Tensor, N: int, c_in: int, c_hid: int) -> int:
    if ab is not None:
        return 0
    if tuple(w2p.shape) != (N, c_hid * c_in) or tuple(b2.shape) != (N, c_hid) or w2p.dtype != torch.bfloat16:
        raise ValueError(f"norm-folded mixer operands must be w2n (N, C_hid*C_in) bf16 and b2n (N, C_hid); got {tuple(w2p.shape)} "
                         f"{w2p.dtype} / {tuple(b2.shape)}")
    return 1


def pw_mlp(t: torch.Tensor, ab: Optional[torch.Tensor], w2p: torch.Tensor, b2: torch.Tensor, w3p: torch.Tensor,
           b3: torch.Tensor, *, N: int, rows_per_sample: int, c_in: int, c_hid: int, c_out: int,
           res: Optional[torch.Tensor] = None, res_mode: int = nat.RES_NONE, grid: Sequence[int] = (0, 0, 0),
           res_low: Optional[torch.Tensor] = None, res_bias: Optional[torch.Tensor] = None,
           y: Optional[torch.Tensor] = None, hidden_pre: Optional[torch.Tensor] = None, lds: bool = False,
           chunked: bool = False, train_nostore: bool = False) -> torch.Tensor:
    _dev(t, "t")
    if t.dtype != torch.bfloat16:
        raise TypeError("pw_mlp runs on bfloat16 activations")
    if y is None:
        y = torch.empty((N, rows_per_sample, c_out), dtype=torch.bfloat16, device=t.device)
    else:
        _check_out(y, N * rows_per_sample * c_out, torch.bfloat16, "pw_mlp")
    a = nat.MlpArgs()
    a.t, a.ab, a.w2_packed, a.b2, a.w3_packed, a.b3 = (t.data_ptr(), None if ab is None else ab.data_ptr(), w2p.data_ptr(),
                                                       b2.data_ptr(), w3p.data_ptr(), b3.data_ptr())
    a.per_sample = _folded_operands(ab, w2p, b2, N, c_in, c_hid)
    a.w3_format = _w3_format(w3p)
    a.res = res.data_ptr() if res is not None else None
    a.res_low = res_low.data_ptr() if res_low is not None else None
    a.res_bias = res_bias.data_ptr() if res_bias is not None else None
    a.y = y.data_ptr()
    a.N, a.rows_per_sample, a.C_in, a.C_hid, a.C_out, a.res_mode = N, rows_per_sample, c_in, c_hid, c_out, res_mode
    a.Di, a.Hi, a.Wi = (int(v) for v in grid)
    nb = N * rows_per_sample * 2 * (c_in + c_out + (c_out if res is not None else 0))
    if hidden_pre is not None:
        _dev(hidden_pre, "hidden_pre")
        _run(f"pw_mlp_train_fwd[{c_in}->{c_hid}->{c_out}]", nb + N * rows_per_sample * 2 * c_hid, nat.lib().pytc_pw_mlp_train_fwd,
             C.byref(a), _p(hidden_pre), _stream())
        return y
# ... 2021 lines not shown
```

pytorch_connectomics_amd/models/architectures/mednext.py:

```python
from __future__ import annotations

import os
from typing import Dict, List, Optional, Sequence, Union

import torch
import torch.nn as nn

from ... import _native as nat
from ... import hip_ops as ops

SMALL_ROWS_TWO_GEMMS = int(os.environ.get("PYTC_MIXER_TWO_GEMM_ROWS", "0"))

L0_SUBBATCH = int(os.environ.get("PYTC_L0_SUBBATCH", "0"))


def _conv_nd(dim: str):
    if dim == "3d":
        return nn.Conv3d, nn.ConvTranspose3d
    if dim == "2d":
        return nn.Conv2d, nn.ConvTranspose2d
    raise ValueError(f"dim must be '2d' or '3d', got {dim!r}")


class _ChannelLayerNorm(nn.Module):

    def __init__(self, normalized_shape: int, eps: float = 1e-5):
        super().__init__()
        self.weight = nn.Parameter(torch.ones(normalized_shape))
        self.bias = nn.Parameter(torch.zeros(normalized_shape))
        self.eps = eps


class MedNeXtBlock(nn.Module):
    def __init__(self, in_channels: int, out_channels: int, exp_r: int = 4, kernel_size: int = 7,
                 do_res: bool = True, norm_type: str = "group", n_groups: Optional[int] = None,
                 dim: str = "3d", grn: bool = False):
        super().__init__()
        conv, _ = _conv_nd(dim)
        self.do_res = do_res
        self.dim = dim
        self.grn = grn
        self.conv1 = conv(in_channels, in_channels, kernel_size=kernel_size, stride=1,
                          padding=kernel_size // 2, groups=in_channels if n_groups is None else n_groups)
        if norm_type == "group":
            self.norm = nn.GroupNorm(num_groups=in_channels, num_channels=in_channels)
        elif norm_type == "layer":
            self.norm = _ChannelLayerNorm(in_channels)
        else:
            raise ValueError(f"norm_type must be 'group' or 'layer', got {norm_type!r}")
        self.conv2 = conv(in_channels, exp_r * in_channels, kernel_size=1, stride=1, padding=0)
        self.act = nn.GELU()
        self.conv3 = conv(exp_r * in_channels, out_channels, kernel_size=1, stride=1, padding=0)
        if grn:
            shape = (1, exp_r * in_channels, 1, 1, 1) if dim == "3d" else (1, exp_r * in_channels, 1, 1)
            self.grn_beta = nn.Parameter(torch.zeros(shape))
            self.grn_gamma = nn.Parameter(torch.zeros(shape))
        self.kind = "block"

    def forward(self, x, dummy_tensor=None):
        raise RuntimeError("MedNeXt blocks execute through MedNeXt.forward (HIP engine); they are parameter "
                           "holders and cannot be called directly")


class MedNeXtDownBlock(MedNeXtBlock):
    def __init__(self, in_channels, out_channels, exp_r=4, kernel_size=7, do_res=False, norm_type="group",
                 dim="3d", grn=False):
        super().__init__(in_channels, out_channels, exp_r, kernel_size, do_res=False, norm_type=norm_type,
                         dim=dim, grn=grn)
        conv, _ = _conv_nd(dim)
        self.resample_do_res = do_res
        if do_res:
            self.res_conv = conv(in_channels, out_channels, kernel_size=1, stride=2)
        self.conv1 = conv(in_channels, in_channels, kernel_size=kernel_size, stride=2,
                          padding=kernel_size // 2, groups=in_channels)
        self.kind = "down"


class MedNeXtUpBlock(MedNeXtBlock):
    def __init__(self, in_channels, out_channels, exp_r=4, kernel_size=7, do_res=False, norm_type="group",
                 dim="3d", grn=False):
        super().__init__(in_channels, out_channels, exp_r, kernel_size, do_res=False, norm_type=norm_type,
                         dim=dim, grn=grn)
        _, convt = _conv_nd(dim)
        self.resample_do_res = do_res
        if do_res:
            self.res_conv = convt(in_channels, out_channels, kernel_size=1, stride=2)
        self.conv1 = convt(in_channels, in_channels, kernel_size=kernel_size, stride=2,
                           padding=kernel_size // 2, groups=in_channels)
        self.kind = "up"


class OutBlock(nn.Module):
    def __init__(self, in_channels: int, n_classes: int, dim: str = "3d"):
        super().__init__()
        _, convt = _conv_nd(dim)
        self.conv_out = convt(in_channels, n_classes, kernel_size=1)

    def forward(self, x, dummy_tensor=None):
        raise RuntimeError("OutBlock executes through MedNeXt.forward (HIP engine)")


class _WeightCache:

    def __init__(self):
        self._store: Dict = {}

    def get(self, key, params: Sequence[torch.Tensor], make):
        sig = tuple((p.data_ptr(), p._version) for p in params)
        hit = self._store.get(key)
        if hit is not None and hit[0] == sig:
            return hit[1]
        with torch.no_grad():
            val = make()
        self._store[key] = (sig, val)
        return val

    def clear(self):
        self._store.clear()


def _f32(p: Optional[torch.Tensor]) -> Optional[torch.Tensor]:
    return None if p is None else p.detach().float().contiguous()


class HipBlockOps:

    def __init__(self):
        self.cache = _WeightCache()
        self.fused = True
        self.fuse_up = os.environ.get("PYTC_FUSE_UP", "0") == "1"
        self.fuse_up_cin = (64, 128)
        self.fold_norm = os.environ.get("PYTC_FOLD_NORM", "1") != "0"
        self.deep_gemm_rows = int(os.environ.get("PYTC_DEEP_GEMM_ROWS", "8192"))
        self.deep_gemm_cin = int(os.environ.get("PYTC_DEEP_GEMM_CIN", "0"))
        self.lds_mixer_rows = int(os.environ.get("PYTC_LDS_MIXER_ROWS", "131072"))
        self.chunk_mixer_rows = int(os.environ.get("PYTC_CHUNK_MIXER_ROWS", "16384"))
        self.chunk_mixer_hid = int(os.environ.get("PYTC_CHUNK_MIXER_HID", "512"))
        self.fuse_block = int(os.environ.get("PYTC_FUSE_BLOCK", "0"))

    def _taps(self, conv: nn.Module):
        w = conv.weight
        def make():
            c = w.shape[0]
            k = w.shape[-1]
            w3 = embed_stencil_2d(w.detach().float()) if w.dim() == 4 else w.detach().float()
            return w3.reshape(c, k ** 3).t().contiguous(), k
        return self.cache.get(("taps", id(conv)), [w], make)

    def _pw(self, conv: nn.Module, dt: torch.dtype, transposed: bool = False):
        w = conv.weight
        def make():
            w2 = w.detach().float().reshape(w.shape[0], w.shape[1]).contiguous()
            return ops.pw_pack_weight(w2, dt, transposed=transposed)
        return self.cache.get(("pw", id(conv), dt, transposed), [w], make)

    def _pw_paired(self, conv: nn.Module, transposed: bool = False, project: bool = False):
        w = conv.weight
        f16 = bool(project and ops.MLP_F16_PROJECT)
        def make():
            w2 = w.detach().float().reshape(w.shape[0], w.shape[1]).contiguous()
            return ops.pw_pack_weight_paired(w2, transposed=transposed, f16=f16)
        return self.cache.get(("pwp", id(conv), transposed, f16), [w], make)

    def _w2_matrix(self, conv: nn.Module):
        w = conv.weight
        return self.cache.get(("w2mat", id(conv)), [w], lambda: w.detach().float().reshape(w.shape[0], w.shape[1]).contiguous())

    def _fold(self, m, st, count, C: int, c_hid: int):
        gamma, beta = self._vec(m.norm, "weight", m.norm.weight), self._vec(m.norm, "bias", m.norm.bias)
        if self.fold_norm and ops.groupnorm_fold_mlp_supported(C, c_hid):
            w2n, b2n = ops.groupnorm_fold_mlp(st, count, gamma, beta, m.norm.eps, self._w2_matrix(m.conv2),
                                              self._vec(m.conv2, "bias", m.conv2.bias))
            return None, w2n, b2n
        return (ops.groupnorm_finalize(st, count, gamma, beta, m.norm.eps), self._pw_paired(m.conv2),
                self._vec(m.conv2, "bias", m.conv2.bias))

    def _head_w(self, conv: nn.Module):
        w = conv.weight
        def make():
            return ops.pack_head_fragment(w.detach().float().reshape(w.shape[0], w.shape[1]).t().contiguous())
        return self.cache.get(("headw", id(conv)), [w], make)

    def _grn(self, m, h: torch.Tensor, N: int, grid, c_hid: int, kind: str) -> torch.Tensor:
        Do, Ho, Wo = grid
        hv = h.view(N, Do, Ho, Wo, c_hid)
        core = hv[:, 1:, 1:, 1:].contiguous() if kind == "up" else hv
        sumsq = ops.channel_stats(core)[:, :, 1].sum(1)
        gx = sumsq.clamp_min(0).sqrt()
        nx = gx / (gx.mean(1, keepdim=True) + 1e-6)
        g = self._vec(m, "grn_gamma", m.grn_gamma).view(1, c_hid)
        b = self._vec(m, "grn_beta", m.grn_beta).view(1, c_hid)
        ab = torch.stack([g * nx + 1.0, b.expand(N, c_hid)], 1).contiguous()
        return ops.affine_act(hv, ab, nat.ACT_NONE, 0.0).view(N, Do * Ho * Wo, c_hid)

    def _vec(self, owner, name: str, p: Optional[torch.Tensor]):
        if p is None:
            return None
        return self.cache.get(("vec", id(owner), name), [p], lambda: _f32(p).reshape(-1))

    def pointwise(self, x: torch.Tensor, conv: nn.Module, *, out_dtype=None, transposed=False, act=nat.ACT_NONE):
        N = x.shape[0]
        spatial = tuple(x.shape[1:-1])
        rows = 1
        for s in spatial:
            rows *= s
        c_in = x.shape[-1]
        c_out = conv.weight.shape[1] if transposed else conv.weight.shape[0]
        dt = x.dtype if x.dtype == torch.bfloat16 else torch.float32
        wdt = torch.bfloat16 if (dt == torch.bfloat16 or (out_dtype == torch.bfloat16)) else torch.float32
        wp = self._pw(conv, wdt, transposed)
        y = ops.pw_conv(x, wp, self._vec(conv, "bias", conv.bias), N=N, rows_per_sample=rows, c_in=c_in,
                        c_out=c_out, out_dtype=out_dtype or x.dtype, act=act)
        return y.view(N, *spatial, c_out)

    def block(self, m: MedNeXtBlock, x: torch.Tensor, skip: Optional[torch.Tensor] = None, head: Optional[nn.Module] = None,
              out: Optional[torch.Tensor] = None, proj: Optional[nn.Module] = None):
        if m.dim == "2d":
            if x.shape[1] != 1:
                raise ValueError(f"dim='2d' MedNeXt blocks take depth-1 volumes (N, 1, H, W, C), got {tuple(x.shape)}")
            if m.kind == "up":
                sk3 = None
                if skip is not None:
                    sk3 = skip.new_zeros((skip.shape[0], 2) + tuple(skip.shape[2:]))
                    sk3[:, 1] = skip[:, 0]
                y = self._block(m, x, sk3, None)[:, 1:2].contiguous()
                return y if out is None else out.copy_(y)
        return self._block(m, x, skip, head, out, proj)

    def _block(self, m: MedNeXtBlock, x: torch.Tensor, skip: Optional[torch.Tensor] = None, head: Optional[nn.Module] = None,
               out: Optional[torch.Tensor] = None, proj: Optional[nn.Module] = None):
        y = self._block_any(m, x, skip, head, out, proj)
        if out is None or isinstance(y, tuple) or y is out:
            return y
        if y.data_ptr() == out.data_ptr():
            return out
        return out.copy_(y.view(out.shape))

    def _block_any(self, m: MedNeXtBlock, x: torch.Tensor, skip: Optional[torch.Tensor] = None, head: Optional[nn.Module] = None,
                   out: Optional[torch.Tensor] = None, proj: Optional[nn.Module] = None):
        is_ln = isinstance(m.norm, _ChannelLayerNorm)
        if not is_ln and not isinstance(m.norm, nn.GroupNorm):
            raise NotImplementedError(f"unsupported MedNeXt norm module {type(m.norm).__name__}")
        dt = x.dtype
        N, D, H, W, C = x.shape
        taps, K = self._taps(m.conv1)
        b1 = self._vec(m.conv1, "bias", m.conv1.bias)
        kind = m.kind
        c_hid = m.conv2.weight.shape[0]
        c_out = m.conv3.weight.shape[0]
        if (kind == "up" and self.fused and self.fuse_up and C in self.fuse_up_cin and dt == torch.bfloat16 and K == 3 and not m.grn and not is_ln
                and m.dim == "3d"
                and skip is not None and m.conv2.bias is not None and m.conv3.bias is not None
                and ops.pw_mlp_up_supported(C, c_hid, c_out)):
            return self._up_block_fused(m, x, skip, taps, b1, c_hid, c_out)
        if (kind == "block" and self.fused and self.fuse_block and self.fold_norm and dt == torch.bfloat16 and K == 3 and not m.grn and not is_ln
                and m.dim == "3d" and m.conv2.bias is not None and m.conv3.bias is not None and ops.MLP_F16_PROJECT
                and ops.dwmix_supported(x, c_hid, c_out) and ops.groupnorm_fold_mlp_supported(C, c_hid)
                and proj is None
                and (head is None or (head.weight.shape[1] <= 16 and ops.pw_mlp_head_supported(C, c_hid, c_out)))):
            return self._block_dwmix(m, x, taps, b1, c_hid, c_out, head, out)
        if kind == "up":
            t, st = ops.dwconv3d(x, taps, b1, K=K, transposed=True, stats=not is_ln)
            count = float((2 * D - 1) * (2 * H - 1) * (2 * W - 1))
        else:
            t, st = ops.dwconv3d(x, taps, b1, K=K, stride=2 if kind == "down" else 1, stats=not is_ln)
            count = float(t.shape[1] * t.shape[2] * t.shape[3])
        gamma, beta = self._vec(m.norm, "weight", m.norm.weight), self._vec(m.norm, "bias", m.norm.bias)
        if is_ln:
            t = ops.layernorm_rows(t, gamma, beta, m.norm.eps)
            ab = None
        else:
            ab = None
        _, Do, Ho, Wo, _ = t.shape
        rows = Do * Ho * Wo
        small = (self.fused and dt == torch.bfloat16 and not m.grn and not is_ln and N * rows < SMALL_ROWS_TWO_GEMMS
                 and ops.pw_conv_paired_supported(c_in=C, c_out=c_hid, in_dtype=dt, out_dtype=dt)
                 and ops.pw_conv_paired_supported(c_in=c_hid, c_out=c_out, in_dtype=dt, out_dtype=dt))
        if (not small and self.fused and dt == torch.bfloat16 and not m.grn and not is_ln and m.conv2.bias is not None
                and m.conv3.bias is not None and head is None and ops.MLP_F16_PROJECT
                and (rows <= self.deep_gemm_rows or (self.deep_gemm_cin and C >= self.deep_gemm_cin))
                and ops.pw_gemm_supported(C, c_hid) and ops.pw_gemm_supported(c_hid, c_out)):
            ab = ops.groupnorm_finalize(st, count, gamma, beta, m.norm.eps)
            return self._block_deep_gemm(m, x, t, ab, skip, (N, D, H, W, C), (Do, Ho, Wo), c_hid, c_out, out)
        if (not small and self.fused and dt == torch.bfloat16 and not m.grn and not is_ln and m.conv2.bias is not None
                and m.conv3.bias is not None and ops.pw_mlp_supported(C, c_hid, c_out)):
            ab, w2x, b2x = self._fold(m, st, count, C, c_hid)
            if (head is not None and kind == "block" and head.weight.shape[1] <= 16
                    and ops.pw_mlp_head_supported(C, c_hid, c_out)):
                _, logits = ops.pw_mlp_head(t, ab, w2x, b2x,
                                            self._pw_paired(m.conv3, project=True), self._vec(m.conv3, "bias", m.conv3.bias),
                                            self._head_w(head), self._vec(head, "bias", head.bias), N=N,
                                            rows_per_sample=rows, c_in=C, c_hid=c_hid, c_out=c_out,
                                            res=x if m.do_res else None, store_y=False)
                return None, logits.view(N, Do, Ho, Wo, -1)
            if (proj is not None and head is None and out is None and kind == "block" and ab is None and ops.MLP_F16_PROJECT
                    and tuple(proj.weight.shape[:2]) == (32, c_out) and ops.pw_mlp_proj_supported(C, c_hid, c_out, 32)):
                _, z = ops.pw_mlp_proj(t, w2x, b2x, self._pw_paired(m.conv3, project=True), self._vec(m.conv3, "bias", m.conv3.bias),
                                       self._pw_paired(proj), self._vec(proj, "bias", proj.bias), N=N, rows_per_sample=rows, c_in=C,
                                       c_hid=c_hid, c_out=c_out, res=x if m.do_res else None, store_y=False)
                return None, z.view(N, Do, Ho, Wo, 32)
            return self._block_fused(m, x, t, ab, skip, (N, D, H, W, C), (Do, Ho, Wo), c_hid, c_out, out, w2x, b2x)
        if not is_ln:
            ab = ops.groupnorm_finalize(st, count, gamma, beta, m.norm.eps)
        G = {}
        if small:
            h = ops.pw_conv(t, self._pw_paired(m.conv2), self._vec(m.conv2, "bias", m.conv2.bias), N=N, rows_per_sample=rows,
                            c_in=C, c_out=c_hid, out_dtype=dt, ab=ab, w_paired=True)
            w3, b3 = self._pw_paired(m.conv3), self._vec(m.conv3, "bias", m.conv3.bias)
            G = dict(pre_act=nat.ACT_GELU, w_paired=True)
        else:
            h = ops.pw_conv(t, self._pw(m.conv2, dt), self._vec(m.conv2, "bias", m.conv2.bias), N=N,
                            rows_per_sample=rows, c_in=C, c_out=c_hid, out_dtype=dt, ab=ab, act=nat.ACT_GELU)
            if m.grn:
                h = self._grn(m, h, N, (Do, Ho, Wo), c_hid, kind)
            w3, b3 = self._pw(m.conv3, dt), self._vec(m.conv3, "bias", m.conv3.bias)
        if kind == "block":
            y = ops.pw_conv(h, w3, b3, N=N, rows_per_sample=rows, c_in=c_hid, c_out=c_out, out_dtype=dt,
                            res=x if m.do_res else None, res_mode=nat.RES_ADD if m.do_res else nat.RES_NONE, **G)
        elif kind == "down":
            res = None
            if m.resample_do_res:
                res = ops.pw_conv(x, self._pw(m.res_conv, dt), self._vec(m.res_conv, "bias", m.res_conv.bias),
                                  N=N, rows_per_sample=rows, c_in=C, c_out=c_out, out_dtype=dt, gather=2,
                                  grid=(D, H, W))
            y = ops.pw_conv(h, w3, b3, N=N, rows_per_sample=rows, c_in=c_hid, c_out=c_out, out_dtype=dt,
                            res=res, res_mode=nat.RES_ADD if res is not None else nat.RES_NONE, **G)
        else:
            if skip is None:
                skip = torch.zeros((N, Do, Ho, Wo, c_out), dtype=dt, device=x.device)
            res_low = res_bias = None
            if m.resample_do_res:
                res_bias = self._vec(m.res_conv, "bias", m.res_conv.bias)
                res_low = ops.pw_conv(x, self._pw(m.res_conv, dt, transposed=True), res_bias, N=N,
                                      rows_per_sample=D * H * W, c_in=C, c_out=c_out, out_dtype=dt)
            y = ops.pw_conv(h, w3, b3, N=N, rows_per_sample=rows, c_in=c_hid, c_out=c_out, out_dtype=dt,
                            res=skip, res_mode=nat.RES_UPSAMPLE, grid=(Do, Ho, Wo), res_low=res_low,
                            res_bias=res_bias, **G)
        return y.view(N, Do, Ho, Wo, c_out)


def _block_dwmix(self, m, x, taps, b1, c_hid, c_out, head=None, out=None):
    N, D, H, W, C = x.shape
    _, st = ops.dwconv3d(x, taps, b1, K=3, store=False)
    w2n, b2n = ops.groupnorm_fold_mlp(st, float(D * H * W), self._vec(m.norm, "weight", m.norm.weight), self._vec(m.norm, "bias", m.norm.bias),
                                      m.norm.eps, self._w2_matrix(m.conv2), self._vec(m.conv2, "bias", m.conv2.bias))
    w3, b3 = self._pw_paired(m.conv3, project=True), self._vec(m.conv3, "bias", m.conv3.bias)
    if head is not None:
        _, logits = ops.dwmix(x, taps, b1, w2n, b2n, w3, b3, c_hid=c_hid, c_out=c_out, residual=bool(m.do_res),
                              head_w=self._head_w(head), head_b=self._vec(head, "bias", head.bias), store_y=False)
        return None, logits
    if out is not None and tuple(out.shape) != (N, D, H, W, c_out):
        raise ValueError(f"block output buffer {tuple(out.shape)} != {(N, D, H, W, c_out)}")
    return ops.dwmix(x, taps, b1, w2n, b2n, w3, b3, c_hid=c_hid, c_out=c_out, residual=bool(m.do_res), y=out)


HipBlockOps._block_dwmix = None


def _stem_block_fused(self, stem: nn.Module, m, x_cl: torch.Tensor, out: Optional[torch.Tensor] = None) -> Optional[torch.Tensor]:
    N, D, H, W, cin = x_cl.shape
    C = stem.weight.shape[0]
    K = m.conv1.weight.shape[-1]
    if (cin != 1 or x_cl.dtype != torch.float32 or stem.bias is None or m.kind != "block" or not m.do_res or m.grn
            or not isinstance(m.norm, nn.GroupNorm) or m.dim != "3d" or m.conv2.bias is None or m.conv3.bias is None
            or m.conv1.weight.shape[0] != C or W % 4 != 0 or not ops.stem_dwconv3d_supported(cin, C, K)):
        return None
    c_hid, c_out = m.conv2.weight.shape[0], m.conv3.weight.shape[0]
    if c_out != C or not ops.pw_mlp_supported(C, c_hid, c_out):
        return None
    sw = self.cache.get(("stemw", id(stem)), [stem.weight], lambda: stem.weight.detach().float().reshape(-1).bfloat16().float().contiguous())
    sb = self._vec(stem, "bias", stem.bias)
    taps, _ = self._taps(m.conv1)
    packed = self.cache.get(("stemdw", id(stem), id(m.conv1)), [stem.weight, stem.bias, m.conv1.weight, m.conv1.bias],
                            lambda: ops.stem_dwconv3d_pack(sw, sb, taps, self._vec(m.conv1, "bias", m.conv1.bias)))
    t, st = ops.stem_dwconv3d(x_cl, packed)
    rows = D * H * W
    ab, w2x, b2x = self._fold(m, st, float(rows), C, c_hid)
    y = ops.pw_mlp_stemres(t, ab, w2x, b2x,
                           self._pw_paired(m.conv3, project=True), self._vec(m.conv3, "bias", m.conv3.bias), x_cl.reshape(N, rows), sw, sb,
                           N=N, rows_per_sample=rows, c_in=C, c_hid=c_hid, c_out=c_out,
                           y=None if out is None else out.view(N, rows, c_out))
    return y.view(N, D, H, W, c_out)


HipBlockOps._stem_block_fused = None


def _block_fused(self, m, x, t, ab, skip, ishape, oshape, c_hid, c_out, out=None, w2=None, b2=None):
    N, D, H, W, C = ishape
    Do, Ho, Wo = oshape
    rows = Do * Ho * Wo
    dt = torch.bfloat16
    if w2 is None:
        w2, b2 = self._pw_paired(m.conv2), self._vec(m.conv2, "bias", m.conv2.bias)
    w3, b3 = self._pw_paired(m.conv3, project=True), self._vec(m.conv3, "bias", m.conv3.bias)
    kw = dict(N=N, rows_per_sample=rows, c_in=C, c_hid=c_hid, c_out=c_out)
    if (self.lds_mixer_rows and N * rows >= self.lds_mixer_rows and w3.dtype == torch.float16
            and ops.pw_mlp_lds_supported(C, c_hid, c_out)):
        kw["lds"] = True
    chunk_ok = (self.chunk_mixer_rows and N * rows >= self.chunk_mixer_rows and w3.dtype == torch.float16
                and ops.pw_mlp_chunk_supported(C, c_hid, c_out))
    if chunk_ok and (c_hid >= self.chunk_mixer_hid or (C, c_out) == (128, 64)):
        kw.pop("lds", None)
        kw["chunked"] = True
    if out is not None:
        if tuple(out.shape) != (N, Do, Ho, Wo, c_out):
            raise ValueError(f"block output buffer {tuple(out.shape)} != {(N, Do, Ho, Wo, c_out)}")
        kw["y"] = out.view(N, rows, c_out)
    if m.kind == "block":
        y = ops.pw_mlp(t, ab, w2, b2, w3, b3, res=x if m.do_res else None,
                       res_mode=nat.RES_ADD if m.do_res else nat.RES_NONE, **kw)
    elif m.kind == "down":
        res = None
        if m.resample_do_res:
            paired = ops.pw_conv_paired_supported(c_in=C, c_out=c_out, in_dtype=dt, out_dtype=dt, gather=2)
            wres = self._pw_paired(m.res_conv) if paired else self._pw(m.res_conv, dt)
            res = ops.pw_conv(x, wres, self._vec(m.res_conv, "bias", m.res_conv.bias), N=N, rows_per_sample=rows,
                              c_in=C, c_out=c_out, out_dtype=dt, gather=2, grid=(D, H, W), w_paired=paired)
        y = ops.pw_mlp(t, ab, w2, b2, w3, b3, res=res, res_mode=nat.RES_ADD if res is not None else nat.RES_NONE, **kw)
    else:
        if skip is None:
            skip = torch.zeros((N, Do, Ho, Wo, c_out), dtype=dt, device=x.device)
        res_low = res_bias = None
        if m.resample_do_res:
            res_bias = self._vec(m.res_conv, "bias", m.res_conv.bias)
            paired = ops.pw_conv_paired_supported(c_in=C, c_out=c_out, in_dtype=dt, out_dtype=dt)
            wres = self._pw_paired(m.res_conv, transposed=True) if paired else self._pw(m.res_conv, dt, transposed=True)
            res_low = ops.pw_conv(x, wres, res_bias, N=N, rows_per_sample=D * H * W, c_in=C, c_out=c_out,
                                  out_dtype=dt, w_paired=paired)
        y = ops.pw_mlp(t, ab, w2, b2, w3, b3, res=skip, res_mode=nat.RES_UPSAMPLE, grid=(Do, Ho, Wo),
                       res_low=res_low, res_bias=res_bias, **kw)
    return y.view(N, Do, Ho, Wo, c_out)


def _block_deep_gemm(self, m, x, t, ab, skip, ishape, oshape, c_hid, c_out, out=None):
    N, D, H, W, C = ishape
    Do, Ho, Wo = oshape
    rows = Do * Ho * Wo
    dt = torch.bfloat16
    w2 = self.cache.get(("gw2", id(m.conv2)), [m.conv2.weight],
                        lambda: m.conv2.weight.detach().float().reshape(c_hid, C).to(torch.bfloat16).contiguous())
    w3 = self.cache.get(("gw3", id(m.conv3)), [m.conv3.weight],
                        lambda: m.conv3.weight.detach().float().reshape(c_out, c_hid).to(torch.float16).contiguous())
    b2, b3 = self._vec(m.conv2, "bias", m.conv2.bias), self._vec(m.conv3, "bias", m.conv3.bias)
    h = ops.pw_gemm(t.view(N, rows, C), w2, b2, N=N, rows_per_sample=rows, ab=ab, gelu=True)
    kw = dict(N=N, rows_per_sample=rows)
    if out is not None:
        kw["y"] = out.view(N, rows, c_out)
    if m.kind == "block":
        y = ops.pw_gemm(h, w3, b3, res=x if m.do_res else None, res_mode=nat.RES_ADD if m.do_res else nat.RES_NONE, **kw)
    elif m.kind == "down":
        res = None
        if m.resample_do_res:
            paired = ops.pw_conv_paired_supported(c_in=C, c_out=c_out, in_dtype=dt, out_dtype=dt, gather=2)
            wres = self._pw_paired(m.res_conv) if paired else self._pw(m.res_conv, dt)
            res = ops.pw_conv(x, wres, self._vec(m.res_conv, "bias", m.res_conv.bias), N=N, rows_per_sample=rows,
                              c_in=C, c_out=c_out, out_dtype=dt, gather=2, grid=(D, H, W), w_paired=paired)
        y = ops.pw_gemm(h, w3, b3, res=res, res_mode=nat.RES_ADD if res is not None else nat.RES_NONE, **kw)
    else:
        if skip is None:
            skip = torch.zeros((N, Do, Ho, Wo, c_out), dtype=dt, device=x.device)
        res_low = res_bias = None
        if m.resample_do_res:
            res_bias = self._vec(m.res_conv, "bias", m.res_conv.bias)
            paired = ops.pw_conv_paired_supported(c_in=C, c_out=c_out, in_dtype=dt, out_dtype=dt)
            wres = self._pw_paired(m.res_conv, transposed=True) if paired else self._pw(m.res_conv, dt, transposed=True)
            res_low = ops.pw_conv(x, wres, res_bias, N=N, rows_per_sample=D * H * W, c_in=C, c_out=c_out, out_dtype=dt, w_paired=paired)
        y = ops.pw_gemm(h, w3, b3, res=skip, res_mode=nat.RES_UPSAMPLE, grid=(Do, Ho, Wo), res_low=res_low, res_bias=res_bias, **kw)
    return y.view(N, Do, Ho, Wo, c_out)


def _up_block_fused(self, m, x, skip, taps, b1, c_hid, c_out):
    N, D, H, W, C = x.shape
    dt = torch.bfloat16
    _, st = ops.dwconv3d(x, taps, b1, K=3, transposed=True, stats=True, store=False)
    ab = ops.groupnorm_finalize(st, float((2 * D - 1) * (2 * H - 1) * (2 * W - 1)), self._vec(m.norm, "weight", m.norm.weight),
                                self._vec(m.norm, "bias", m.norm.bias), m.norm.eps)
    res_low = res_bias = None
    if m.resample_do_res:
        res_bias = self._vec(m.res_conv, "bias", m.res_conv.bias)
        paired = ops.pw_conv_paired_supported(c_in=C, c_out=c_out, in_dtype=dt, out_dtype=dt)
        wres = self._pw_paired(m.res_conv, transposed=True) if paired else self._pw(m.res_conv, dt, transposed=True)
        res_low = ops.pw_conv(x, wres, res_bias, N=N, rows_per_sample=D * H * W, c_in=C, c_out=c_out, out_dtype=dt,
                              w_paired=paired)
    return ops.pw_mlp_up(x, taps, b1, ab, self._pw_paired(m.conv2), self._vec(m.conv2, "bias", m.conv2.bias),
                         self._pw_paired(m.conv3), self._vec(m.conv3, "bias", m.conv3.bias), skip.contiguous(),
                         c_hid=c_hid, c_out=c_out, res_low=res_low, res_bias=res_bias)


HipBlockOps._up_block_fused = _up_block_fused
HipBlockOps._block_deep_gemm = _block_deep_gemm
HipBlockOps._block_fused = _block_fused
HipBlockOps._stem_block_fused = _stem_block_fused
HipBlockOps._block_dwmix = _block_dwmix


def resolve_compute_dtype(module_pref: Optional[torch.dtype]) -> torch.dtype:
    if module_pref is not None:
        return module_pref
    if torch.is_autocast_enabled("cuda"):
        adt = torch.get_autocast_dtype("cuda")
        if adt == torch.bfloat16:
            return torch.bfloat16
        if adt == torch.float16:
            raise RuntimeError("fp16 autocast is not supported by the MI355X engine; use bf16-mixed")
    return torch.float32


def embed_stencil_2d(w: torch.Tensor) -> torch.Tensor:
    k = w.shape[-1]
    out = w.new_zeros((w.shape[0], w.shape[1], k, k, k))
    out[:, :, k // 2] = w
    return out


def to_channels_last(x: torch.Tensor) -> torch.Tensor:
    if x.shape[1] == 1:
        return x.reshape(x.shape[0], *x.shape[2:], 1)
    return x.permute(0, 2, 3, 4, 1).contiguous()


def to_channels_first(y: torch.Tensor) -> torch.Tensor:
    if y.shape[-1] == 1:
        return y.reshape(y.shape[0], 1, *y.shape[1:-1])
    return y.permute(0, 4, 1, 2, 3).contiguous()


class MedNeXt(nn.Module):

    def __init__(self, in_channels: int, n_channels: int, n_classes: int, exp_r: Union[int, Sequence[int]] = 4,
                 kernel_size: int = 7, enc_kernel_size: Optional[int] = None,
                 dec_kernel_size: Optional[int] = None, deep_supervision: bool = False, do_res: bool = False,
                 do_res_up_down: bool = False, checkpoint_style: Optional[str] = None,
                 block_counts: Sequence[int] = (2, 2, 2, 2, 2, 2, 2, 2, 2), norm_type: str = "group",
                 dim: str = "3d", grn: bool = False):
        super().__init__()
        if checkpoint_style not in (None, "outside_block"):
            raise ValueError("checkpoint_style must be None or 'outside_block'")
        if len(block_counts) != 9:
            raise ValueError("block_counts must have exactly 9 elements")
        self.do_ds = deep_supervision
        self.inside_block_checkpointing = False
        self.outside_block_checkpointing = checkpoint_style == "outside_block"
        self.checkpoint_policy = "auto"
        if kernel_size is not None:
            enc_kernel_size = dec_kernel_size = kernel_size
        conv, _ = _conv_nd(dim)
        if isinstance(exp_r, int):
            exp_r = [exp_r] * 9
        exp_r = list(exp_r)
        n = n_channels
        self.dim = dim
        self.stem = conv(in_channels, n, kernel_size=1)

        def blocks(c, r, k, count):
            return nn.Sequential(*[MedNeXtBlock(c, c, r, k, do_res, norm_type, dim=dim, grn=grn)
                                   for _ in range(count)])

        for lvl in range(4):
            setattr(self, f"enc_block_{lvl}", blocks(n << lvl, exp_r[lvl], enc_kernel_size, block_counts[lvl]))
            setattr(self, f"down_{lvl}", MedNeXtDownBlock(n << lvl, n << (lvl + 1), exp_r[lvl + 1], enc_kernel_size,
                                                          do_res=do_res_up_down, norm_type=norm_type, dim=dim, grn=grn))
        self.bottleneck = blocks(n << 4, exp_r[4], dec_kernel_size, block_counts[4])
        for i, lvl in enumerate((3, 2, 1, 0)):
            setattr(self, f"up_{lvl}", MedNeXtUpBlock(n << (lvl + 1), n << lvl, exp_r[5 + i], dec_kernel_size,
                                                      do_res=do_res_up_down, norm_type=norm_type, dim=dim, grn=grn))
            setattr(self, f"dec_block_{lvl}", blocks(n << lvl, exp_r[5 + i], dec_kernel_size, block_counts[5 + i]))
        self.out_0 = OutBlock(n, n_classes, dim)
        self.dummy_tensor = nn.Parameter(torch.tensor([1.0]), requires_grad=True)
        if deep_supervision:
            for h in (1, 2, 3, 4):
                setattr(self, f"out_{h}", OutBlock(n << h, n_classes, dim))
        self.block_counts = list(block_counts)
        self.compute_dtype: Optional[torch.dtype] = None
        self._hip = HipBlockOps()
        self.fuse_head = True
        self.fuse_stem = True
        self.l0_subbatch = L0_SUBBATCH

    def _check_input(self, x: torch.Tensor):
        if not x.is_cuda:
            raise RuntimeError("MedNeXt (pytorch_connectomics_amd) runs only on an MI355X/ROCm device: "
                               "there is no CPU path. Move the model and input to 'cuda'.")
        if self.dim == "2d":
            if x.dim() not in (4, 5) or (x.dim() == 5 and x.shape[2] != 1):
                raise ValueError(f"MedNeXt dim='2d' takes (B,C,H,W) (or (B,C,1,H,W)) inputs, got {tuple(x.shape)}")
        elif x.dim() != 5:
            raise ValueError(f"MedNeXt dim='3d' takes (B,C,D,H,W) inputs, got {tuple(x.shape)}")
        spatial = x.shape[-2:] if self.dim == "2d" else x.shape[2:]
        if any(int(v) % 16 for v in spatial):
            raise ValueError(f"MedNeXt needs spatial sizes divisible by 16, got {tuple(spatial)}")

    def _lift(self, x: torch.Tensor):
        if self.dim == "2d" and x.dim() == 4:
            return x.unsqueeze(2), True
        return x, False

    @staticmethod
    def _drop(y, was_4d: bool):
        if not was_4d:
            return y
        if isinstance(y, list):
            return [v.squeeze(2) for v in y]
        return y.squeeze(2)

    def features_cl(self, x_cl: torch.Tensor, collect: Optional[List[torch.Tensor]] = None,
                    head: Optional[nn.Module] = None, proj: Optional[nn.Module] = None):
        hip = self._hip
        dt = resolve_compute_dtype(self.compute_dtype)
        spatial = x_cl.shape[2:4] if self.dim == "2d" else x_cl.shape[1:4]
        if any(int(v) % 16 for v in spatial) or (self.dim == "2d" and x_cl.shape[1] != 1):
            raise ValueError(f"MedNeXt needs spatial sizes divisible by 16, got {tuple(x_cl.shape[1:4])}"
                             + (" (dim='2d': depth must be 1)" if self.dim == "2d" else ""))
        enc0 = list(self.enc_block_0)
        N = int(x_cl.shape[0])
        sb = int(self.l0_subbatch)
        chained = 0 < sb < N and dt == torch.bfloat16 and hip.fused and self.dim == "3d"
        fuse_stem = self.fuse_stem and hip.fused and dt == torch.bfloat16 and bool(enc0)

        def level0_encoder(xs: torch.Tensor, skip_out: Optional[torch.Tensor], down_out: Optional[torch.Tensor]):
            blocks = list(enc0)
            h = None
            if fuse_stem:
                h = hip._stem_block_fused(self.stem, blocks[0], xs, skip_out if len(blocks) == 1 else None)
                if h is not None:
                    blocks = blocks[1:]
            if h is None:
                h = hip.pointwise(xs, self.stem, out_dtype=dt)
                if not blocks and skip_out is not None:
                    h = skip_out.copy_(h)
            for bi, blk in enumerate(blocks):
                h = hip.block(blk, h, out=skip_out if bi == len(blocks) - 1 else None)
            return h, hip.block(self.down_0, h, out=down_out)

        def level0_decoder(xl: torch.Tensor, sk: torch.Tensor, y_out: Optional[torch.Tensor] = None):
            h = hip.block(self.up_0, xl, skip=sk)
            blocks = list(self.dec_block_0)
            for bi, blk in enumerate(blocks):
                last = bi == len(blocks) - 1
                h = hip.block(blk, h, head=head if last else None, out=y_out if last else None, proj=proj if last else None)
            if not blocks and y_out is not None:
                h = y_out.copy_(h)
            return h

        skips = []
        if chained:
            _, D0, H0, W0, _ = x_cl.shape
            c0, c1 = self.stem.weight.shape[0], self.down_0.conv3.weight.shape[0]
            skip0 = torch.empty((N, D0, H0, W0, c0), dtype=dt, device=x_cl.device)
            x = torch.empty((N, D0 // 2, H0 // 2, W0 // 2, c1), dtype=dt, device=x_cl.device)
            for s0 in range(0, N, sb):
                level0_encoder(x_cl[s0:s0 + sb], skip0[s0:s0 + sb], x[s0:s0 + sb])
            skips.append(skip0)
        else:
            h, x = level0_encoder(x_cl, None, None)
            skips.append(h)
        for lvl in range(1, 4):
            for blk in getattr(self, f"enc_block_{lvl}"):
                x = hip.block(blk, x)
            skips.append(x)
            x = hip.block(getattr(self, f"down_{lvl}"), x)
        for blk in self.bottleneck:
            x = hip.block(blk, x)
        if collect is not None:
            collect.append(x)
        for lvl in (3, 2, 1):
            x = hip.block(getattr(self, f"up_{lvl}"), x, skip=skips[lvl])
            for blk in getattr(self, f"dec_block_{lvl}"):
                x = hip.block(blk, x)
            if collect is not None:
                collect.append(x)
        if not chained:
            return level0_decoder(x, skips[0])
        first = level0_decoder(x[0:sb], skips[0][0:sb])
        if isinstance(first, tuple):
            parts = [first[1]] + [level0_decoder(x[s0:s0 + sb], skips[0][s0:s0 + sb])[1] for s0 in range(sb, N, sb)]
            return None, torch.cat(parts, 0)
        y0 = torch.empty((N,) + tuple(first.shape[1:]), dtype=first.dtype, device=first.device)
        y0[0:sb].copy_(first)
        for s0 in range(sb, N, sb):
            level0_decoder(x[s0:s0 + sb], skips[0][s0:s0 + sb], y0[s0:s0 + sb])
        return y0

    def output_cl(self, feat_cl: torch.Tensor, head: int = 0) -> torch.Tensor:
        return self._hip.pointwise(feat_cl, getattr(self, f"out_{head}").conv_out, out_dtype=torch.float32,
                                   transposed=True)

    def forward_cl(self, x_cl: torch.Tensor):
        out = self.features_cl(x_cl, head=self.out_0.conv_out if self.fuse_head else None)
        if isinstance(out, tuple):
            return out[1]
        return self.output_cl(out)

    def forward_features(self, x: torch.Tensor) -> torch.Tensor:
        self._check_input(x)
        x, flat = self._lift(x)
        return self._drop(to_channels_first(self.features_cl(to_channels_last(x.float())).float()), flat)

    def forward_output(self, features: torch.Tensor) -> torch.Tensor:
        if not features.is_cuda:
            raise RuntimeError("forward_output needs a CUDA tensor: there is no CPU path")
        dt = resolve_compute_dtype(self.compute_dtype)
        features, flat = self._lift(features)
        return self._drop(to_channels_first(self.output_cl(to_channels_last(features).to(dt))), flat)

    def _autograd_active(self) -> bool:
        return torch.is_grad_enabled() and any(p.requires_grad for p in self.parameters())

    def forward(self, x: torch.Tensor):
        self._check_input(x)
        x, flat = self._lift(x)
        return self._drop(self._forward5(x), flat)

    def _forward5(self, x: torch.Tensor):
        if self._autograd_active():
            from ...training.autograd import mednext_train_forward
            out = mednext_train_forward(self, to_channels_last(x.float()), resolve_compute_dtype(self.compute_dtype))
            if isinstance(out, list):
                return [to_channels_first(o) for o in out]
            return to_channels_first(out)
        if not self.do_ds:
            return to_channels_first(self.forward_cl(to_channels_last(x.float())))
        feats: Optional[List[torch.Tensor]] = []
        f = self.features_cl(to_channels_last(x.float()), collect=feats)
        out = to_channels_first(self.output_cl(f))
        ds = [to_channels_first(self.output_cl(ft, h)) for ft, h in zip(feats, (4, 3, 2, 1))]
        return [out, ds[3], ds[2], ds[1], ds[0]]


def create_mednext_v1(num_input_channels: int, num_classes: int, model_id: str, kernel_size: int = 3,
                      deep_supervision: bool = False) -> MedNeXt:
    table = {
        "S": dict(exp_r=2, block_counts=[2] * 9, checkpoint_style=None),
        "B": dict(exp_r=[2, 3, 4, 4, 4, 4, 4, 3, 2], block_counts=[2] * 9, checkpoint_style=None),
        "M": dict(exp_r=[2, 3, 4, 4, 4, 4, 4, 3, 2], block_counts=[3, 4, 4, 4, 4, 4, 4, 4, 3],
                  checkpoint_style="outside_block"),
        "L": dict(exp_r=[3, 4, 8, 8, 8, 8, 8, 4, 3], block_counts=[3, 4, 8, 8, 8, 8, 8, 4, 3],
                  checkpoint_style="outside_block"),
    }
    if model_id not in table:
        raise ValueError(f"model_id must be one of S, B, M, L; got {model_id!r}")
    return MedNeXt(in_channels=num_input_channels, n_channels=32, n_classes=num_classes,
                   kernel_size=kernel_size, deep_supervision=deep_supervision, do_res=True,
                   do_res_up_down=True, **table[model_id])


__all__ = ["MedNeXt", "MedNeXtBlock", "MedNeXtDownBlock", "MedNeXtUpBlock", "OutBlock", "create_mednext_v1",
           "HipBlockOps", "to_channels_last", "to_channels_first", "resolve_compute_dtype"]
```

Before: 1.787 billion voxels/s.

## Fuse residual 1x1 conv into resampling depthwise kernels of down/up blocks

Down and up blocks at the shallow levels now compute the residual 1x1 projection on the matrix cores inside the stride-2 and transposed depthwise tile kernels. Those kernels already hold the input tile in LDS, so the separate residual pw_conv launch and its second read of the input are no longer needed. A new tuning knob (on by default) gates the path, and block scheduling is factored into a helper so the fused residual is used only when the downstream deep or fused MLP path consumes it. The cost is extra register pressure and MFMA work in the depthwise kernels, which may lower their occupancy.

```diff
diff --git a/include/pytc_hip.h b/include/pytc_hip.h
--- a/include/pytc_hip.h
+++ b/include/pytc_hip.h
@@ -7,7 +7,7 @@
 extern "C" {
 #endif
 
-#define PYTC_ABI_VERSION 15
+#define PYTC_ABI_VERSION 16
 
 #define PYTC_OK 0
 #define PYTC_ERR_INVALID 1
@@ -132,8 +132,16 @@
 int pytc_dwconv3d_fwd_res(const void* x, const void* res, void* y, const float* w, const float* bias, int N, int D, int H,
                           int W, int C, int K, int stride, int dtype, void* stream);
 
+int pytc_dwconv3d_s2_res_supported(int D, int H, int W, int C, int dtype);
+int pytc_dwconv3d_s2_res_fwd(const void* x, void* y, const float* w, const float* bias, float* stats, const void* res_w,
+                             const float* res_bias, void* res, int N, int D, int H, int W, int C, int dtype, void* stream);
+
 int pytc_dwconvT3d_fwd(const void* x, void* y, const float* w, const float* bias, float* stats,
                        int N, int D, int H, int W, int C, int K, int dtype, void* stream);
+
+int pytc_dwconvT3d_res_supported(int D, int H, int W, int C, int dtype);
+int pytc_dwconvT3d_res_fwd(const void* x, void* y, const float* w, const float* bias, float* stats, const void* res_w,
+                           const float* res_bias, void* res_low, int N, int D, int H, int W, int C, int dtype, void* stream);
 
 int pytc_groupnorm_finalize(const float* stats, int slots, float count, const float* gamma,
                             const float* beta, float eps, float* ab, int N, int C, void* stream);
diff --git a/pytorch_connectomics_amd/csrc/dwconvT_tile_kernels.hip b/pytorch_connectomics_amd/csrc/dwconvT_tile_kernels.hip
--- a/pytorch_connectomics_amd/csrc/dwconvT_tile_kernels.hip
+++ b/pytorch_connectomics_amd/csrc/dwconvT_tile_kernels.hip
@@ -1,15 +1,22 @@
 #include <mutex>
 
 #include "dwconv_march.h"
+#include "pw_common.h"
 
 namespace pytc {
 
+struct TTRes {
+  const bf16x8_t* w;
+  const float* bias;
+  bf16_t* res;
+};
+
 constexpr int TT_TZ = 2, TT_TX = 8;
 
-template <int C, int TY, bool STORE>
+template <int C, int TY, bool STORE, bool RES = false>
 __global__ void __launch_bounds__(256, 4)
 dwconvT3d_k3_tile_kernel(const unsigned short* __restrict__ x, unsigned short* __restrict__ y, const float* __restrict__ w,
-                         const float* __restrict__ bias, float* __restrict__ stats, DwTTile g) {
+                         const float* __restrict__ bias, float* __restrict__ stats, DwTTile g, TTRes rp) {
   constexpr int LPV = C / 2;
   constexpr int SLOTS = 256 / LPV;
   constexpr int CELLS = TT_TZ * TY * TT_TX;
@@ -58,6 +65,41 @@
     if (c < NCH) *reinterpret_cast<u32x4_t*>(tile + (long)c * 8) = st[i];
   }
   __syncthreads();
+
+  if (RES) {
+    constexpr int RKS = C / 32, RCO = C / 2, RPAIRS = RCO / 32, NTW = CELLS / 16 / 4;
+    static_assert(CELLS % 64 == 0, "whole MFMA tiles per wave");
+    const int rlane = tid & 63, rr = rlane & 15, rkb = rlane >> 4;
+    bf16_t* const resn = rp.res + (long)n * vcells * RCO;
+#pragma unroll
+    for (int j = 0; j < NTW; ++j) {
+      const int cell = ((tid >> 6) * NTW + j) * 16 + rr;
+      const int cx = cell % TT_TX, t = cell / TT_TX;
+      const int cy = t % TY, cz = t / TY;
+      const int mz = z0 + cz, my = y0 + cy, mx = x0 + cx;
+      const bool live = mz < g.D && my < g.H && mx < g.W;
+      const unsigned short* row = tile + (((cz + 1) * EY + cy + 1) * EX + cx + 1) * C + rkb * 8;
+      bf16x8_t rb[RKS];
+#pragma unroll
+      for (int ks = 0; ks < RKS; ++ks) rb[ks] = *reinterpret_cast<const bf16x8_t*>(row + ks * 32);
+#pragma unroll
+      for (int pq = 0; pq < RPAIRS; ++pq) {
+        const int o0 = pq * 32 + rkb * 8;
+        f32x4_t acc[2];
+#pragma unroll
+        for (int mt = 0; mt < 2; ++mt) {
+          acc[mt] = rp.bias ? *reinterpret_cast<const f32x4_t*>(rp.bias + o0 + mt * 4) : f32x4_t{0.f, 0.f, 0.f, 0.f};
+#pragma unroll
+          for (int ks = 0; ks < RKS; ++ks)
+            acc[mt] = Mma<bf16_t>::mma(rp.w[((pq * 2 + mt) * RKS + ks) * 64 + rlane], rb[ks], acc[mt]);
+        }
+        float v[8];
+#pragma unroll
+        for (int q = 0; q < 4; ++q) { v[q] = acc[0][q]; v[4 + q] = acc[1][q]; }
+        if (live) VecIO<bf16_t, 8>::store(resn + (((long)mz * g.H + my) * g.W + mx) * RCO + o0, v);
+      }
+    }
+  }
 
   typedef __bf16 bf2_t __attribute__((ext_vector_type(2)));
   typedef float f2_t __attribute__((ext_vector_type(2)));
@@ -167,19 +209,46 @@
   return g.slots >= 1 && (long)D * H * W * 8 * C * 2 < (1L << 32) && (long)(2 * H) * (2 * W) * C * 4 < (1L << 24);
 }
 
-void dwconvT_tile_launch(const void* x, void* y, const float* w, const float* bias, float* stats, const DwTTile& g, hipStream_t s) {
+void dwconvT_tile_launch(const void* x, void* y, const float* w, const float* bias, float* stats, const DwTTile& g, hipStream_t s,
+                         const void* res_w, const float* res_bias, void* res_low) {
   dim3 grid((unsigned)g.slots, (unsigned)g.N), block(256);
   const unsigned short* xp = (const unsigned short*)x;
   unsigned short* yp = (unsigned short*)y;
-#define PYTC_TT(CC, TYY, ST)                                                                                                  \
+  const TTRes rp = {(const bf16x8_t*)res_w, res_bias, (bf16_t*)res_low};
+#define PYTC_TT(CC, TYY, ST, RR)                                                                                              \
   do {                                                                                                                        \
-    if (!ensure_dynamic_lds(reinterpret_cast<const void*>(&dwconvT3d_k3_tile_kernel<CC, TYY, ST>), 64 * 1024, "dwconvT3d_k3_tile")) return; \
-    hipLaunchKernelGGL((dwconvT3d_k3_tile_kernel<CC, TYY, ST>), grid, block,                                                  \
-                       (size_t)(TT_TZ + 1) * (TYY + 1) * (TT_TX + 1) * CC * 2 + 4 * 2048, s, xp, yp, w, bias, stats, g);                  \
+    if (!ensure_dynamic_lds(reinterpret_cast<const void*>(&dwconvT3d_k3_tile_kernel<CC, TYY, ST, RR>), 64 * 1024, "dwconvT3d_k3_tile")) return; \
+    hipLaunchKernelGGL((dwconvT3d_k3_tile_kernel<CC, TYY, ST, RR>), grid, block,                                              \
+                       (size_t)(TT_TZ + 1) * (TYY + 1) * (TT_TX + 1) * CC * 2 + 4 * 2048, s, xp, yp, w, bias, stats, g, rp);              \
   } while (0)
-  if (g.C == 64) { if (y) PYTC_TT(64, 8, true); else PYTC_TT(64, 8, false); }
-  else { if (y) PYTC_TT(128, 4, true); else PYTC_TT(128, 4, false); }
+  if (res_low && y) {
+    if (g.C == 64) PYTC_TT(64, 8, true, true);
+    else PYTC_TT(128, 4, true, true);
+  } else if (g.C == 64) { if (y) PYTC_TT(64, 8, true, false); else PYTC_TT(64, 8, false, false); }
+  else { if (y) PYTC_TT(128, 4, true, false); else PYTC_TT(128, 4, false, false); }
 #undef PYTC_TT
 }
 
 }
+
+using namespace pytc;
+
+extern "C" int pytc_dwconvT3d_res_supported(int D, int H, int W, int C, int dtype) {
+  DwTTile g;
+  return dtype == PYTC_BF16 && tuning_get(K_resample_res_fused) != 0 && tuning_get(K_dwconvT_tile) != 0 && D > 0 && H > 0 && W > 0 &&
+         dwconvT_tile_plan(g, 1, D, H, W, C);
+}
+
+extern "C" int pytc_dwconvT3d_res_fwd(const void* x, void* y, const float* w, const float* bias, float* stats, const void* res_w,
+                                      const float* res_bias, void* res_low, int N, int D, int H, int W, int C, int dtype, void* stream) {
+  PYTC_REQUIRE(x && y && w && res_w && res_low, "dwconvT3d_res: null pointer");
+  PYTC_REQUIRE(N >= 1 && pytc_dwconvT3d_res_supported(D, H, W, C, dtype),
+               "dwconvT3d_res: bf16, C = 64 / 128 and the knobs resample_res_fused / dwconvT_tile on (pytc_dwconvT3d_res_supported)");
+  PYTC_REQUIRE((((uintptr_t)res_w | (uintptr_t)res_low | (uintptr_t)res_bias) & 15) == 0,
+               "dwconvT3d_res: the weight image, its bias and the residual output must be 16-byte aligned");
+  DwTTile g;
+  PYTC_REQUIRE(dwconvT_tile_plan(g, N, D, H, W, C), "dwconvT3d_res: shape outside the tile kernel's range");
+  dwconvT_tile_launch(x, y, w, bias, stats, g, (hipStream_t)stream, res_w, res_bias, res_low);
+  PYTC_LAUNCH_CHECK("dwconvT3d_k3_tile");
+  return PYTC_OK;
+}
diff --git a/pytorch_connectomics_amd/csrc/dwconv_march.h b/pytorch_connectomics_amd/csrc/dwconv_march.h
--- a/pytorch_connectomics_amd/csrc/dwconv_march.h
+++ b/pytorch_connectomics_amd/csrc/dwconv_march.h
@@ -32,10 +32,12 @@
 
 struct DwTTile { int N, D, H, W, C, tz, ty, tx, slots; };
 bool dwconvT_tile_plan(DwTTile& g, int N, int D, int H, int W, int C);
-void dwconvT_tile_launch(const void* x, void* y, const float* w, const float* bias, float* stats, const DwTTile& g, hipStream_t s);
+void dwconvT_tile_launch(const void* x, void* y, const float* w, const float* bias, float* stats, const DwTTile& g, hipStream_t s,
+                         const void* res_w = nullptr, const float* res_bias = nullptr, void* res_low = nullptr);
 
 struct DwS2 { int N, D, H, W, C, Do, Ho, Wo, ty, tx, zc, nzc, slots; };
 bool dwconv_s2_plan(DwS2& g, int N, int D, int H, int W, int C);
-void dwconv_s2_launch(const void* x, void* y, const float* w, const float* bias, float* stats, const DwS2& g, hipStream_t s);
+void dwconv_s2_launch(const void* x, void* y, const float* w, const float* bias, float* stats, const DwS2& g, hipStream_t s,
+                      const void* res_w = nullptr, const float* res_bias = nullptr, void* res = nullptr);
 
 }
diff --git a/pytorch_connectomics_amd/csrc/dwconv_s2_kernels.hip b/pytorch_connectomics_amd/csrc/dwconv_s2_kernels.hip
--- a/pytorch_connectomics_amd/csrc/dwconv_s2_kernels.hip
+++ b/pytorch_connectomics_amd/csrc/dwconv_s2_kernels.hip
@@ -1,15 +1,22 @@
 #include <mutex>
 
 #include "dwconv_march.h"
+#include "pw_common.h"
 
 namespace pytc {
 
+struct S2Res {
+  const bf16x8_t* w;
+  const float* bias;
+  bf16_t* res;
+};
+
 constexpr int S2_TYO = 4;
 
-template <int C>
+template <int C, bool RES = false>
 __global__ void __launch_bounds__(256, 2)
 dwconv3d_k3_s2_march_kernel(const unsigned short* __restrict__ x, unsigned short* __restrict__ y, const float* __restrict__ w,
-                            const float* __restrict__ bias, float* __restrict__ stats, DwS2 g) {
+                            const float* __restrict__ bias, float* __restrict__ stats, DwS2 g, S2Res rp) {
   constexpr int TYO = S2_TYO, TXO = 8, IY = 2 * TYO + 1, IX = 2 * TXO + 1;
   constexpr int LPV = C / 2, VS = 256 / LPV, OUTV = TYO * TXO, ITEMS = OUTV / VS;
   constexpr int PCH = IY * IX * (C / 8);
@@ -75,6 +82,31 @@
   const bool ook = tid < OPIECES && oyy < g.Ho && oxx < g.Wo;
   const long obase = ((long)oyy * g.Wo + oxx) * C + opart * 8;
 
+  constexpr int RKS = C / 32, RCO = 2 * C, RPW = RCO / 32 / 2;
+  const int rlane = tid & 63, rr = rlane & 15, rkb = rlane >> 4;
+  const int rv = ((tid >> 6) & 1) * 16 + rr, rp0 = (tid >> 7) * RPW;
+  const int rvy = rv / TXO, rvx = rv % TXO;
+  const int rboff = ((2 * rvy + 1) * IX + 2 * rvx + 1) * C + rkb * 8;
+  const bool rlive = RES && (yo0 + rvy) < g.Ho && (xo0 + rvx) < g.Wo;
+  bf16x8_t ra[RES ? RPW : 1][2][RKS];
+  f32x4_t rbias[RES ? RPW : 1][2];
+  long roff = 0;
+  if (RES) {
+#pragma unroll
+    for (int q = 0; q < RPW; ++q) {
+#pragma unroll
+      for (int mt = 0; mt < 2; ++mt)
+#pragma unroll
+        for (int ks = 0; ks < RKS; ++ks) ra[q][mt][ks] = rp.w[((long)((rp0 + q) * 2 + mt) * RKS + ks) * 64 + rlane];
+      rbias[q][0] = rbias[q][1] = f32x4_t{0.f, 0.f, 0.f, 0.f};
+      if (rp.bias) {
+        rbias[q][0] = *reinterpret_cast<const f32x4_t*>(rp.bias + (rp0 + q) * 32 + rkb * 8);
+        rbias[q][1] = *reinterpret_cast<const f32x4_t*>(rp.bias + (rp0 + q) * 32 + rkb * 8 + 4);
+      }
+    }
+    roff = (long)n * g.Do * g.Ho * g.Wo * RCO + ((long)(yo0 + rvy) * g.Wo + (xo0 + rvx)) * RCO + rp0 * 32 + rkb * 8;
+  }
+
   u32x4_t sa[LPT], sb[LPT];
   request(2 * zs - 1, sa);
   request(2 * zs, sb);
@@ -91,6 +123,23 @@
     const unsigned short* p0 = ring + ((2 * zo) % 3) * PLANE;
     const unsigned short* p1 = ring + ((2 * zo + 1) % 3) * PLANE;
     const unsigned short* p2 = ring + ((2 * zo + 2) % 3) * PLANE;
+    if (RES) {
+      bf16x8_t rb[RKS];
+#pragma unroll
+      for (int ks = 0; ks < RKS; ++ks) rb[ks] = *reinterpret_cast<const bf16x8_t*>(p1 + rboff + ks * 32);
+#pragma unroll
+      for (int q = 0; q < RPW; ++q) {
+        f32x4_t acc[2] = {rbias[q][0], rbias[q][1]};
+#pragma unroll
+        for (int mt = 0; mt < 2; ++mt)
+#pragma unroll
+          for (int ks = 0; ks < RKS; ++ks) acc[mt] = Mma<bf16_t>::mma(ra[q][mt][ks], rb[ks], acc[mt]);
+        float v[8];
+#pragma unroll
+        for (int j = 0; j < 4; ++j) { v[j] = acc[0][j]; v[4 + j] = acc[1][j]; }
+        if (rlive) VecIO<bf16_t, 8>::store(rp.res + roff + (long)zo * g.Ho * g.Wo * RCO + q * 32, v);
+      }
+    }
 #pragma unroll
     for (int it = 0; it < ITEMS; ++it) {
       const int v = vslot + it * VS;
@@ -161,19 +210,46 @@
   return (long)H * W * C < (1L << 30);
 }
 
-void dwconv_s2_launch(const void* x, void* y, const float* w, const float* bias, float* stats, const DwS2& g, hipStream_t s) {
+void dwconv_s2_launch(const void* x, void* y, const float* w, const float* bias, float* stats, const DwS2& g, hipStream_t s,
+                      const void* res_w, const float* res_bias, void* res) {
   dim3 grid((unsigned)g.slots, (unsigned)g.N), block(256);
   const unsigned short* xp = (const unsigned short*)x;
   unsigned short* yp = (unsigned short*)y;
-#define PYTC_S2(CC)                                                                                                           \
+  const S2Res rp = {(const bf16x8_t*)res_w, res_bias, (bf16_t*)res};
+#define PYTC_S2(CC, RR)                                                                                                         \
   do {                                                                                                                        \
     const size_t lds = (size_t)(3 * (2 * S2_TYO + 1) * 17 * CC + S2_TYO * 8 * CC) * 2;                                         \
-    if (!ensure_dynamic_lds(reinterpret_cast<const void*>(&dwconv3d_k3_s2_march_kernel<CC>), 72 * 1024, "dwconv3d_k3_s2_march")) return; \
-    hipLaunchKernelGGL((dwconv3d_k3_s2_march_kernel<CC>), grid, block, lds, s, xp, yp, w, bias, stats, g);                    \
+    if (!ensure_dynamic_lds(reinterpret_cast<const void*>(&dwconv3d_k3_s2_march_kernel<CC, RR>), 72 * 1024, "dwconv3d_k3_s2_march")) return; \
+    hipLaunchKernelGGL((dwconv3d_k3_s2_march_kernel<CC, RR>), grid, block, lds, s, xp, yp, w, bias, stats, g, rp);        \
   } while (0)
-  if (g.C == 32) PYTC_S2(32);
-  else PYTC_S2(64);
+  if (res) {
+    if (g.C == 32) PYTC_S2(32, true);
+    else PYTC_S2(64, true);
+  } else if (g.C == 32) PYTC_S2(32, false);
+  else PYTC_S2(64, false);
 #undef PYTC_S2
 }
 
 }
+
+using namespace pytc;
+
+extern "C" int pytc_dwconv3d_s2_res_supported(int D, int H, int W, int C, int dtype) {
+  DwS2 g;
+  return dtype == PYTC_BF16 && tuning_get(K_resample_res_fused) != 0 && tuning_get(K_dwconv_s2_march) != 0 && D > 0 && H > 0 && W > 0 &&
+         dwconv_s2_plan(g, 1, D, H, W, C);
+}
+
+extern "C" int pytc_dwconv3d_s2_res_fwd(const void* x, void* y, const float* w, const float* bias, float* stats, const void* res_w,
+                                        const float* res_bias, void* res, int N, int D, int H, int W, int C, int dtype, void* stream) {
+  PYTC_REQUIRE(x && y && w && res_w && res, "dwconv3d_s2_res: null pointer");
+  PYTC_REQUIRE(N >= 1 && pytc_dwconv3d_s2_res_supported(D, H, W, C, dtype),
+               "dwconv3d_s2_res: bf16, C = 32 / 64 and the knobs resample_res_fused / dwconv_s2_march on (pytc_dwconv3d_s2_res_supported)");
+  PYTC_REQUIRE((((uintptr_t)res_w | (uintptr_t)res | (uintptr_t)res_bias) & 15) == 0,
+               "dwconv3d_s2_res: the weight image, its bias and the residual output must be 16-byte aligned");
+  DwS2 g;
+  dwconv_s2_plan(g, N, D, H, W, C);
+  dwconv_s2_launch(x, y, w, bias, stats, g, (hipStream_t)stream, res_w, res_bias, res);
+  PYTC_LAUNCH_CHECK("dwconv3d_k3_s2_march");
+  return PYTC_OK;
+}
diff --git a/pytorch_connectomics_amd/csrc/pytc_common.h b/pytorch_connectomics_amd/csrc/pytc_common.h
--- a/pytorch_connectomics_amd/csrc/pytc_common.h
+++ b/pytorch_connectomics_amd/csrc/pytc_common.h
@@ -82,6 +82,7 @@
   X(norm_bwd_from_wgrad_flat, 1, "GroupNorm-backward epilogue of the expand weight gradient as one flat kernel; 0 = chunked")      \
   X(pw_gemm_rows, 0, "LDS-tiled 1x1 GEMM: 64 / 128 forces the rows per workgroup; 0 = by problem size")                            \
   X(pw_thin, 1, "plain 1x1 convs with one input / few output channels on the thin kernels; 0 = the generic kernel")                \
+  X(resample_res_fused, 1, "down / up blocks (bf16, levels 0 / 1): residual 1x1 conv inside the resampling depthwise kernel; 0 = own launch") \
   X(wgrad_dgrad_fused, 1, "projecting conv's weight gradient and the GELU-backward data gradient in one kernel; 0 = two launches")  \
   X(wgrad_small_split, 1, "matrix-core 1x1 weight gradient: more, shorter row slots when the launch would leave CUs idle")         \
   X(wgrad_valu, 0, "1: 1x1 weight gradient on the VALU kernel instead of the matrix cores")                                        \
diff --git a/pytorch_connectomics_amd/hip_ops.py b/pytorch_connectomics_amd/hip_ops.py
--- a/pytorch_connectomics_amd/hip_ops.py
+++ b/pytorch_connectomics_amd/hip_ops.py
@@ -306,7 +306,7 @@
 
 def dwconv3d(x: torch.Tensor, w_taps: torch.Tensor, bias: Optional[torch.Tensor], *, K: int, stride: int = 1,
              stats: bool = True, transposed: bool = False, y: Optional[torch.Tensor] = None, store: bool = True,
-             wide_range: bool = False):
+             wide_range: bool = False, res_w: Optional[torch.Tensor] = None, res_bias: Optional[torch.Tensor] = None):
     _dev(x, "x"); _dev(w_taps, "w_taps")
     N, D, H, W, Cc = x.shape
     dt = dtype_code(x.dtype)
@@ -328,6 +328,24 @@
             raise RuntimeError(f"dwconv3d: unsupported channel count {Cc}")
         st = torch.empty((N, slots, 2, Cc), dtype=torch.float32, device=x.device)
     tag = f"C{Cc}_k{K}" + ("_s2" if stride == 2 and not transposed else "")
+    if res_w is not None:
+        _dev(res_w, "res_w")
+        if not (store and K == 3 and (transposed or stride == 2) and not wide_range
+                and dwconv3d_res_conv_supported(x, transposed=transposed)):
+            raise ValueError("dwconv3d(res_w=...): no fused residual conv for this launch (dwconv3d_res_conv_supported)")
+        c_res = Cc // 2 if transposed else 2 * Cc
+        if res_w.dtype != torch.bfloat16 or res_w.numel() != c_res * Cc or (res_bias is not None and (
+                res_bias.dtype != torch.float32 or res_bias.numel() != c_res or not res_bias.is_cuda)):
+            raise ValueError(f"dwconv3d(res_w=...): paired bf16 image of [{c_res}][{Cc}] and an fp32 bias of {c_res} expected")
+        if transposed:
+            res = torch.empty((N, D, H, W, c_res), dtype=x.dtype, device=x.device)
+            _run(f"dwconvT3d_res_conv[{tag}]", _nbytes(x, y, res), nat.lib().pytc_dwconvT3d_res_fwd, _p(x), _p(y), _p(w_taps), _p(bias),
+                 _p(st), _p(res_w), _p(res_bias), _p(res), N, D, H, W, Cc, dt, _stream(), symbol="dwconvT3d_k3_tile_kernel")
+        else:
+            res = torch.empty(oshape[:4] + (c_res,), dtype=x.dtype, device=x.device)
+            _run(f"dwconv3d_res_conv[{tag}]", _nbytes(x, y, res), nat.lib().pytc_dwconv3d_s2_res_fwd, _p(x), _p(y), _p(w_taps), _p(bias),
+                 _p(st), _p(res_w), _p(res_bias), _p(res), N, D, H, W, Cc, dt, _stream(), symbol="dwconv3d_k3_s2_march_kernel")
+        return y, st, res
     if transposed:
         _run(f"dwconvT3d_fwd[{tag}]" if store else f"dwconvT3d_stats[{tag}]", _nbytes(x, y), nat.lib().pytc_dwconvT3d_fwd, _p(x), _p(y), _p(w_taps), _p(bias),
              _p(st), N, D, H, W, Cc, K, dt, _stream())
@@ -344,6 +362,17 @@
 _DW_VARIANTS = {0: "dwconv3d_direct_kernel", 1: "dwconv3d_k3_gather_kernel", 2: "dwconv3d_xblock_kernel",
                 3: "dwconv3d_k3_march_kernel", 4: "dwconvT3d_k3_cell_kernel", 5: "dwconvT3d_kernel",
                 6: "dwconv3d_k3_mfma_kernel", 7: "dwconvT3d_k3_tile_kernel", 8: "dwconv3d_k3_s2_march_kernel"}
+
+
+def dwconv3d_res_conv_supported(x: torch.Tensor, K: int = 3, *, transposed: bool = False) -> bool:
+    N, D, H, W, Cc = x.shape
+    if K != 3 or x.dtype != torch.bfloat16:
+        return False
+    if transposed:
+        return bool(nat.lib().pytc_dwconvT3d_res_supported(D, H, W, Cc, dtype_code(x.dtype))) and pw_conv_paired_supported(
+            c_in=Cc, c_out=Cc // 2, in_dtype=x.dtype, out_dtype=x.dtype)
+    return bool(nat.lib().pytc_dwconv3d_s2_res_supported(D, H, W, Cc, dtype_code(x.dtype))) and pw_conv_paired_supported(
+        c_in=Cc, c_out=2 * Cc, in_dtype=x.dtype, out_dtype=x.dtype, gather=2)
 
 
 def dwconv3d_res_supported(x: torch.Tensor, K: int, stride: int = 1) -> bool:
diff --git a/pytorch_connectomics_amd/models/architectures/mednext.py b/pytorch_connectomics_amd/models/architectures/mednext.py
--- a/pytorch_connectomics_amd/models/architectures/mednext.py
+++ b/pytorch_connectomics_amd/models/architectures/mednext.py
@@ -236,6 +236,28 @@
             return out
         return out.copy_(y.view(out.shape))
 
+    def _schedule(self, m, total_rows: int, rows: int, C: int, dt, is_ln: bool, head, c_hid: int, c_out: int) -> str:
+        bf16 = self.fused and dt == torch.bfloat16 and not m.grn and not is_ln
+        if (bf16 and total_rows < SMALL_ROWS_TWO_GEMMS
+                and ops.pw_conv_paired_supported(c_in=C, c_out=c_hid, in_dtype=dt, out_dtype=dt)
+                and ops.pw_conv_paired_supported(c_in=c_hid, c_out=c_out, in_dtype=dt, out_dtype=dt)):
+            return "small"
+        if not bf16 or m.conv2.bias is None or m.conv3.bias is None:
+            return "plain"
+        if (head is None and ops.MLP_F16_PROJECT
+                and (rows <= self.deep_gemm_rows or (self.deep_gemm_cin and C >= self.deep_gemm_cin))
+                and ops.pw_gemm_supported(C, c_hid) and ops.pw_gemm_supported(c_hid, c_out)):
+            return "deep"
+        return "fused" if ops.pw_mlp_supported(C, c_hid, c_out) else "plain"
+
+    def _resample_takes_paired_res(self, m, x: torch.Tensor, is_ln: bool, head, c_hid: int, c_out: int) -> bool:
+        N, D, H, W, C = x.shape
+        if m.kind == "up":
+            rows = 8 * D * H * W
+        else:
+            rows = ((D - 1) // 2 + 1) * ((H - 1) // 2 + 1) * ((W - 1) // 2 + 1)
+        return self._schedule(m, N * rows, rows, C, x.dtype, is_ln, head, c_hid, c_out) in ("deep", "fused")
+
     def _block_any(self, m: MedNeXtBlock, x: torch.Tensor, skip: Optional[torch.Tensor] = None, head: Optional[nn.Module] = None,
                    out: Optional[torch.Tensor] = None, proj: Optional[nn.Module] = None):
         is_ln = isinstance(m.norm, _ChannelLayerNorm)
@@ -259,9 +281,21 @@
                 and proj is None
                 and (head is None or (head.weight.shape[1] <= 16 and ops.pw_mlp_head_supported(C, c_hid, c_out)))):
             return self._block_dwmix(m, x, taps, b1, c_hid, c_out, head, out)
-        if kind == "up":
+        res_pre = None
+        fuse_res = (kind in ("down", "up") and K == 3 and m.dim == "3d" and m.resample_do_res
+                    and self._resample_takes_paired_res(m, x, is_ln, head, c_hid, c_out)
+                    and ops.dwconv3d_res_conv_supported(x, transposed=kind == "up"))
+        if kind == "up" and fuse_res:
+            t, st, res_pre = ops.dwconv3d(x, taps, b1, K=K, transposed=True, stats=True, res_w=self._pw_paired(m.res_conv, transposed=True),
+                                          res_bias=self._vec(m.res_conv, "bias", m.res_conv.bias))
+            count = float((2 * D - 1) * (2 * H - 1) * (2 * W - 1))
+        elif kind == "up":
             t, st = ops.dwconv3d(x, taps, b1, K=K, transposed=True, stats=not is_ln)
             count = float((2 * D - 1) * (2 * H - 1) * (2 * W - 1))
+        elif fuse_res:
+            t, st, res_pre = ops.dwconv3d(x, taps, b1, K=K, stride=2, stats=True, res_w=self._pw_paired(m.res_conv),
+                                          res_bias=self._vec(m.res_conv, "bias", m.res_conv.bias))
+            count = float(t.shape[1] * t.shape[2] * t.shape[3])
         else:
             t, st = ops.dwconv3d(x, taps, b1, K=K, stride=2 if kind == "down" else 1, stats=not is_ln)
             count = float(t.shape[1] * t.shape[2] * t.shape[3])
@@ -273,17 +307,12 @@
             ab = None
         _, Do, Ho, Wo, _ = t.shape
         rows = Do * Ho * Wo
-        small = (self.fused and dt == torch.bfloat16 and not m.grn and not is_ln and N * rows < SMALL_ROWS_TWO_GEMMS
-                 and ops.pw_conv_paired_supported(c_in=C, c_out=c_hid, in_dtype=dt, out_dtype=dt)
-                 and ops.pw_conv_paired_supported(c_in=c_hid, c_out=c_out, in_dtype=dt, out_dtype=dt))
-        if (not small and self.fused and dt == torch.bfloat16 and not m.grn and not is_ln and m.conv2.bias is not None
-                and m.conv3.bias is not None and head is None and ops.MLP_F16_PROJECT
-                and (rows <= self.deep_gemm_rows or (self.deep_gemm_cin and C >= self.deep_gemm_cin))
-                and ops.pw_gemm_supported(C, c_hid) and ops.pw_gemm_supported(c_hid, c_out)):
+        schedule = self._schedule(m, N * rows, rows, C, dt, is_ln, head, c_hid, c_out)
+        small = schedule == "small"
+        if schedule == "deep":
             ab = ops.groupnorm_finalize(st, count, gamma, beta, m.norm.eps)
-            return self._block_deep_gemm(m, x, t, ab, skip, (N, D, H, W, C), (Do, Ho, Wo), c_hid, c_out, out)
-        if (not small and self.fused and dt == torch.bfloat16 and not m.grn and not is_ln and m.conv2.bias is not None
-                and m.conv3.bias is not None and ops.pw_mlp_supported(C, c_hid, c_out)):
+            return self._block_deep_gemm(m, x, t, ab, skip, (N, D, H, W, C), (Do, Ho, Wo), c_hid, c_out, out, res=res_pre)
+        if schedule == "fused":
             ab, w2x, b2x = self._fold(m, st, count, C, c_hid)
             if (head is not None and kind == "block" and head.weight.shape[1] <= 16
                     and ops.pw_mlp_head_supported(C, c_hid, c_out)):
@@ -299,7 +328,7 @@
                                        self._pw_paired(proj), self._vec(proj, "bias", proj.bias), N=N, rows_per_sample=rows, c_in=C,
                                        c_hid=c_hid, c_out=c_out, res=x if m.do_res else None, store_y=False)
                 return None, z.view(N, Do, Ho, Wo, 32)
-            return self._block_fused(m, x, t, ab, skip, (N, D, H, W, C), (Do, Ho, Wo), c_hid, c_out, out, w2x, b2x)
+            return self._block_fused(m, x, t, ab, skip, (N, D, H, W, C), (Do, Ho, Wo), c_hid, c_out, out, w2x, b2x, res=res_pre)
         if not is_ln:
             ab = ops.groupnorm_finalize(st, count, gamma, beta, m.norm.eps)
         G = {}
@@ -386,7 +415,7 @@
 HipBlockOps._stem_block_fused = None
 
 
-def _block_fused(self, m, x, t, ab, skip, ishape, oshape, c_hid, c_out, out=None, w2=None, b2=None):
+def _block_fused(self, m, x, t, ab, skip, ishape, oshape, c_hid, c_out, out=None, w2=None, b2=None, res=None):
     N, D, H, W, C = ishape
     Do, Ho, Wo = oshape
     rows = Do * Ho * Wo
@@ -411,8 +440,7 @@
         y = ops.pw_mlp(t, ab, w2, b2, w3, b3, res=x if m.do_res else None,
                        res_mode=nat.RES_ADD if m.do_res else nat.RES_NONE, **kw)
     elif m.kind == "down":
-        res = None
-        if m.resample_do_res:
+        if m.resample_do_res and res is None:
             paired = ops.pw_conv_paired_supported(c_in=C, c_out=c_out, in_dtype=dt, out_dtype=dt, gather=2)
             wres = self._pw_paired(m.res_conv) if paired else self._pw(m.res_conv, dt)
             res = ops.pw_conv(x, wres, self._vec(m.res_conv, "bias", m.res_conv.bias), N=N, rows_per_sample=rows,
@@ -421,9 +449,10 @@
     else:
         if skip is None:
             skip = torch.zeros((N, Do, Ho, Wo, c_out), dtype=dt, device=x.device)
-        res_low = res_bias = None
+        res_low, res_bias = res, None
         if m.resample_do_res:
             res_bias = self._vec(m.res_conv, "bias", m.res_conv.bias)
+        if m.resample_do_res and res_low is None:
             paired = ops.pw_conv_paired_supported(c_in=C, c_out=c_out, in_dtype=dt, out_dtype=dt)
             wres = self._pw_paired(m.res_conv, transposed=True) if paired else self._pw(m.res_conv, dt, transposed=True)
             res_low = ops.pw_conv(x, wres, res_bias, N=N, rows_per_sample=D * H * W, c_in=C, c_out=c_out,
@@ -433,7 +462,7 @@
     return y.view(N, Do, Ho, Wo, c_out)
 
 
-def _block_deep_gemm(self, m, x, t, ab, skip, ishape, oshape, c_hid, c_out, out=None):
+def _block_deep_gemm(self, m, x, t, ab, skip, ishape, oshape, c_hid, c_out, out=None, res=None):
     N, D, H, W, C = ishape
     Do, Ho, Wo = oshape
     rows = Do * Ho * Wo
@@ -450,8 +479,7 @@
     if m.kind == "block":
         y = ops.pw_gemm(h, w3, b3, res=x if m.do_res else None, res_mode=nat.RES_ADD if m.do_res else nat.RES_NONE, **kw)
     elif m.kind == "down":
-        res = None
-        if m.resample_do_res:
+        if m.resample_do_res and res is None:
             paired = ops.pw_conv_paired_supported(c_in=C, c_out=c_out, in_dtype=dt, out_dtype=dt, gather=2)
             wres = self._pw_paired(m.res_conv) if paired else self._pw(m.res_conv, dt)
             res = ops.pw_conv(x, wres, self._vec(m.res_conv, "bias", m.res_conv.bias), N=N, rows_per_sample=rows,
@@ -460,9 +488,10 @@
     else:
         if skip is None:
             skip = torch.zeros((N, Do, Ho, Wo, c_out), dtype=dt, device=x.device)
-        res_low = res_bias = None
+        res_low, res_bias = res, None
         if m.resample_do_res:
             res_bias = self._vec(m.res_conv, "bias", m.res_conv.bias)
+        if m.resample_do_res and res_low is None:
             paired = ops.pw_conv_paired_supported(c_in=C, c_out=c_out, in_dtype=dt, out_dtype=dt)
             wres = self._pw_paired(m.res_conv, transposed=True) if paired else self._pw(m.res_conv, dt, transposed=True)
             res_low = ops.pw_conv(x, wres, res_bias, N=N, rows_per_sample=D * H * W, c_in=C, c_out=c_out, out_dtype=dt, w_paired=paired)
```

Measured after the change: 1.811 billion voxels/s (median of 6 runs). 1.4% higher.
